# angeris/cfmm-routing-code

Measured on AMD Instinct MI355X. Metric: pool-subproblems/sec to 1e-6 rel-gap; 1e6 pools / 1k tokens; 1/2/4/8 GPU, higher is better.
Workload: dtype f64; 1 GPU; C3: 1000000 pools per GPU (cp2=700000, w2=200000, gn3-8=100000) / 1000 tokens, linear-utility arbitrage, cold-start solve to gap,infeas <= 1e-06; pools_per_gpu=1000000, pools_total=1000000, seed=0, parallelism=single GPU, rccl_ranks=1

## Files before the change

cfmm-routing-code_amd/csrc/cfmm_hip.hip:

```cpp
#include <hip/hip_runtime.h>
#include <dlfcn.h>
#include <algorithm>
#include <cmath>
#include <atomic>
#include <chrono>
#include <condition_variable>
#include <cstdarg>
#include <cstdio>
#include <cstdlib>
#include <cstring>
#include <map>
#include <memory>
#include <set>
#include <mutex>
#include <functional>
#include <limits>
#include <string>
#include <thread>
#include <type_traits>
#include <vector>

#include "../../include/cfmm.h"
#include "kernels.hpp"
#include "iterate.hpp"
// ... 413 lines not shown
            if (!got) {
                std::unique_lock<std::mutex> g(mu_);
                cv_.wait(g, [&]() { return gen_.load(std::memory_order_acquire) != seen; });
            }
            seen = gen_.load(std::memory_order_acquire);
            { std::lock_guard<std::mutex> g(mu_); if (!job_) continue; active_.fetch_add(1, std::memory_order_relaxed); }
            work();
            active_.fetch_sub(1, std::memory_order_release);
        }
    }
    std::mutex mu_, run_mu_;
    std::condition_variable cv_;
    const std::function<void(int)> *job_ = nullptr;
    int njobs_ = 0, nthreads_ = 0;
    std::atomic<int> next_{0}, left_{0}, active_{0};
    std::atomic<unsigned long long> gen_{0};
};

struct UploadScan {
    std::atomic<bool> bad{false};
    std::mutex mu;
    double mxr = 0.0, mnf = 1.0;
    void fold(double mx, double mn) { std::lock_guard<std::mutex> g(mu); mxr = std::max(mxr, mx); mnf = std::min(mnf, mn); }
};
struct Col {
    size_t bytes = 0;
    void **dst = nullptr;
    std::function<void(char *out, size_t off, size_t len)> fill;
    const void *direct = nullptr;
};
template <class F>
void parallel_range(int64_t m, F f)
{
    const int T = m >= (1 << 15) ? HostPool::get().threads() : 1;
    if (T == 1) { f((int64_t)0, m); return; }
    const int64_t part = (m + T - 1) / T;
    HostPool::get().run(T, [&](int t) { const int64_t b = t * part, e = std::min<int64_t>(m, b + part); if (b < e) f(b, e); });
}

template <class T, class P>
inline bool copy_scan(T *out, const T *src, size_t cnt, P pred, T &mx, T &mn)
{
    std::memcpy(out, src, cnt * sizeof(T));
    bool ok0 = true, ok1 = true, ok2 = true, ok3 = true;
    T a0 = mx, a1 = mx, a2 = mx, a3 = mx, b0 = mn, b1 = mn, b2 = mn, b3 = mn;
    size_t i = 0;
    for (; i + 4 <= cnt; i += 4) {
        const T x0 = out[i], x1 = out[i + 1], x2 = out[i + 2], x3 = out[i + 3];
        ok0 &= pred(x0); ok1 &= pred(x1); ok2 &= pred(x2); ok3 &= pred(x3);
        a0 = x0 > a0 ? x0 : a0; a1 = x1 > a1 ? x1 : a1; a2 = x2 > a2 ? x2 : a2; a3 = x3 > a3 ? x3 : a3;
        b0 = x0 < b0 ? x0 : b0; b1 = x1 < b1 ? x1 : b1; b2 = x2 < b2 ? x2 : b2; b3 = x3 < b3 ? x3 : b3;
    }
    for (; i < cnt; ++i) { const T x = out[i]; ok0 &= pred(x); a0 = x > a0 ? x : a0; b0 = x < b0 ? x : b0; }
    mx = std::max(std::max(a0, a1), std::max(a2, a3)); mn = std::min(std::min(b0, b1), std::min(b2, b3));
    return ok0 && ok1 && ok2 && ok3;
}
template <class T, class P>
Col checked_col(const T *src, size_t count, void **dst, UploadScan *scan, int role, P pred)
{
    Col c; c.bytes = count * sizeof(T); c.dst = dst; c.direct = src;
    c.fill = [src, scan, role, pred](char *out, size_t off, size_t len) {
        T mx = T(0), mn = T(1);
        if (role == 2) { mx = std::numeric_limits<T>::lowest(); mn = std::numeric_limits<T>::max(); }
        if (!copy_scan<T>((T *)out, src + off / sizeof(T), len / sizeof(T), pred, mx, mn)) scan->bad.store(true, std::memory_order_relaxed);
        if (role == 0) scan->fold((double)mx, 1.0);
        if (role == 1) scan->fold(0.0, (double)mn);
    };
    return c;
}
Col plain_col(const void *src, size_t bytes, void **dst)
{
    Col c; c.bytes = bytes; c.dst = dst; c.direct = src;
    c.fill = [src](char *out, size_t off, size_t len) { std::memcpy(out, (const char *)src + off, len); };
    return c;
}
template <class T, int K, class P>
inline void transpose_fill(T *o, const T *src, int64_t m, size_t e, size_t cnt, P pred, bool &ok, T &mx)
{
    size_t q = 0;
    int64_t i = (int64_t)(e / K); int j = (int)(e % K);
    for (; q < cnt && j != 0; ++q) { const T x = src[(size_t)j * m + i]; o[q] = x; ok &= pred(x); mx = x > mx ? x : mx; if (++j == K) { j = 0; ++i; } }
    bool okv = true; T mxv = mx;
    for (; q + K <= cnt; q += K, ++i) {
#pragma unroll
        for (int jj = 0; jj < K; ++jj) { const T x = src[(size_t)jj * m + i]; o[q + jj] = x; okv &= pred(x); mxv = x > mxv ? x : mxv; }
    }
    ok &= okv; mx = mxv;
    for (j = 0; q < cnt; ++q, ++j) { const T x = src[(size_t)j * m + i]; o[q] = x; ok &= pred(x); mx = x > mx ? x : mx; }
}
template <class T, class P>
Col transposed_col(const T *src, int k, int64_t m, void **dst, UploadScan *scan, bool track_max, P pred)
{
    Col c; c.bytes = (size_t)k * m * sizeof(T); c.dst = dst;
    c.fill = [src, k, m, scan, track_max, pred](char *out, size_t off, size_t len) {
        T *o = (T *)out;
        const size_t e = off / sizeof(T), cnt = len / sizeof(T);
        bool ok = true; T mx = T(0);
        with_int<2, 8>(k, [&](auto K) { transpose_fill<T, K>(o, src, m, e, cnt, pred, ok, mx); });
        if (!ok) scan->bad.store(true, std::memory_order_relaxed);
        if (track_max) scan->fold((double)mx, 1.0);
    };
    return c;
}
void parallel_fill(const Col &c, char *out, size_t off, size_t len)
{
    const size_t grain = 64u << 10;
    int T = (int)std::min<size_t>((len + grain - 1) / grain, (size_t)HostPool::get().threads());
    if (T <= 1) { c.fill(out, off, len); return; }
    const size_t part = ((len / T) + 63) & ~(size_t)63;
    HostPool::get().run(T, [&](int t) {
        const size_t b = (size_t)t * part, e = (t == T - 1) ? len : std::min(len, b + part);
        if (b < e) c.fill(out + b, off + b, e - b);
    });
}
int upload_arena(cfmm_ctx *ctx, std::vector<Col> &cols, void **arena_out, const UploadScan *scan = nullptr, size_t *total_out = nullptr)
{
    size_t total = 0;
    std::vector<size_t> offs;
    size_t staged = 0;
    for (auto &c : cols) {
        offs.push_back(total); total += (c.bytes + 255) & ~(size_t)255;
        if (c.fill) { if (staged != offs.back()) return fail(ctx, CFMM_E_STATE, "upload: a staged column behind a reserved one"); staged = total; }
    }
    char *base = nullptr;
    static const bool trace = getenv("CFMM_UPLOAD_TRACE") != nullptr;
    auto now = []() { return std::chrono::steady_clock::now(); };
    auto ms = [](std::chrono::steady_clock::time_point a, std::chrono::steady_clock::time_point b) { return std::chrono::duration<double, std::milli>(b - a).count(); };
    const auto tA = now();
    HIP_TRY(ctx, hipMalloc((void **)&base, total + 256));
    if (total_out) *total_out = total;
    const auto tB = now();
    double t_fill = 0.0, t_wait = 0.0, t_enq = 0.0;
    auto bail = [&](hipError_t e, const char *what) { (void)hipStreamSynchronize(ctx->stream); (void)hipFree(base); return fail(ctx, CFMM_E_HIP, "upload: %s -> %s", what, hipGetErrorString(e)); };
    static const bool by_register = getenv("CFMM_UPLOAD") && std::string(getenv("CFMM_UPLOAD")) == "register";
    if (by_register) {
        std::vector<void *> pinned;
        hipError_t e = hipSuccess;
        for (size_t q = 0; q < cols.size() && e == hipSuccess; ++q) {
            if (!cols[q].fill) { *cols[q].dst = base + offs[q]; continue; }
            std::vector<char> tmp(cols[q].bytes);
            cols[q].fill(tmp.data(), 0, cols[q].bytes);
            if (cols[q].direct && cols[q].bytes >= (1u << 20)) {
                e = hipHostRegister(const_cast<void *>(cols[q].direct), cols[q].bytes, hipHostRegisterDefault);
                if (e == hipSuccess) { pinned.push_back(const_cast<void *>(cols[q].direct)); e = hipMemcpyAsync(base + offs[q], cols[q].direct, cols[q].bytes, hipMemcpyHostToDevice, ctx->stream); }
            } else {
                e = hipMemcpy(base + offs[q], tmp.data(), cols[q].bytes, hipMemcpyHostToDevice);
            }
            *cols[q].dst = base + offs[q];
        }
        if (e == hipSuccess) e = hipStreamSynchronize(ctx->stream);
        for (void *h : pinned) (void)hipHostUnregister(h);
        if (e != hipSuccess) return bail(e, "hipHostRegister / copy");
        if (scan && scan->bad.load()) { (void)hipFree(base); return CFMM_E_ARG; }
        *arena_out = base;
        return CFMM_OK;
    }
    std::lock_guard<std::mutex> lock(g_stage.mu);
    if (!g_stage.buf) {
        hipError_t e = hipHostMalloc((void **)&g_stage.buf, STAGE_SLOTS * STAGE_BYTES, hipHostMallocDefault);
        if (e != hipSuccess) { g_stage.buf = nullptr; return bail(e, "hipHostMalloc(staging)"); }
        for (auto &ev : g_stage.ev) { e = hipEventCreateWithFlags(&ev, hipEventDisableTiming); if (e != hipSuccess) return bail(e, "hipEventCreate"); }
    }
    struct Job { size_t q, col_off, len, st_off; };
    int slot = g_stage.next;
    bool *used = g_stage.used;
    std::vector<Job> jobs;
    for (size_t c0 = 0; c0 < staged; c0 += STAGE_BYTES) {
        const size_t clen = std::min(STAGE_BYTES, staged - c0);
        char *st = g_stage.buf + (size_t)slot * STAGE_BYTES;
        jobs.clear();
        for (size_t q = 0; q < cols.size(); ++q) {
            const size_t lo = std::max(offs[q], c0), hi = std::min(offs[q] + cols[q].bytes, c0 + clen);
            if (lo >= hi || !cols[q].fill) continue;
            const size_t grain = 64u << 10;
            for (size_t b = lo; b < hi; b += grain) jobs.push_back({q, b - offs[q], std::min(grain, hi - b), b - c0});
        }
        const auto t0 = now();
        if (used[slot]) { hipError_t e = stage_slot_wait(slot); if (e != hipSuccess) return bail(e, "hipEventSynchronize"); }
        const auto t1 = now();
        HostPool::get().run((int)jobs.size(), [&](int j) { const Job &w = jobs[j]; cols[w.q].fill(st + w.st_off, w.col_off, w.len); });
        const auto t2 = now();
        if (scan && scan->bad.load(std::memory_order_relaxed)) { (void)hipStreamSynchronize(ctx->stream); (void)hipFree(base); return CFMM_E_ARG; }
        hipError_t e = hipMemcpyAsync(base + c0, st, clen, hipMemcpyHostToDevice, ctx->stream);
        if (e == hipSuccess) e = hipEventRecord(g_stage.ev[slot], ctx->stream);
        if (e != hipSuccess) return bail(e, "hipMemcpyAsync");
        t_wait += ms(t0, t1); t_fill += ms(t1, t2); t_enq += ms(t2, now());
        used[slot] = true; g_stage.last[slot] = ctx->stream; slot = (slot + 1) % STAGE_SLOTS;
    }
    for (size_t q = 0; q < cols.size(); ++q) *cols[q].dst = base + offs[q];
    g_stage.next = slot;
    if (trace) fprintf(stderr, "[cfmm upload] %.2f MB: hipMalloc %.3f ms, fill %.3f, wait-for-slot %.3f, enqueue %.3f, total %.3f\n",
                       total / 1e6, ms(tA, tB), t_fill, t_wait, t_enq, ms(tA, now()));
    *arena_out = base;
    return CFMM_OK;
}

int download_staged(cfmm_ctx *ctx, void *host_dst, const void *dev_src, size_t bytes)
{
    if (bytes < (1u << 20)) {
        HIP_TRY(ctx, hipMemcpyAsync(host_dst, dev_src, bytes, hipMemcpyDeviceToHost, ctx->stream));
        HIP_TRY(ctx, hipStreamSynchronize(ctx->stream));
        return CFMM_OK;
    }
    std::lock_guard<std::mutex> lock(g_stage.mu);
    if (!g_stage.buf) {
        HIP_TRY(ctx, hipHostMalloc((void **)&g_stage.buf, STAGE_SLOTS * STAGE_BYTES, hipHostMallocDefault));
        for (auto &ev : g_stage.ev) HIP_TRY(ctx, hipEventCreateWithFlags(&ev, hipEventDisableTiming));
    }
    for (int q = 0; q < STAGE_SLOTS; ++q) if (g_stage.used[q]) { HIP_TRY(ctx, stage_slot_wait(q)); g_stage.used[q] = false; }
    const size_t nchunks = (bytes + STAGE_BYTES - 1) / STAGE_BYTES;
    auto enqueue = [&](size_t c) -> hipError_t {
        const size_t off = c * STAGE_BYTES, len = std::min(STAGE_BYTES, bytes - off);
        const int slot = (int)(c % STAGE_SLOTS);
        hipError_t e = hipMemcpyAsync(g_stage.buf + (size_t)slot * STAGE_BYTES, (const char *)dev_src + off, len, hipMemcpyDeviceToHost, ctx->stream);
        if (e == hipSuccess) e = hipEventRecord(g_stage.ev[slot], ctx->stream);
        return e;
    };
    hipError_t e = hipSuccess;
    for (size_t c = 0; c < std::min<size_t>(nchunks, STAGE_SLOTS - 1) && e == hipSuccess; ++c) e = enqueue(c);
    for (size_t c = 0; c < nchunks && e == hipSuccess; ++c) {
        if (c + STAGE_SLOTS - 1 < nchunks) e = enqueue(c + STAGE_SLOTS - 1);
        if (e != hipSuccess) break;
        const int slot = (int)(c % STAGE_SLOTS);
        e = hipEventSynchronize(g_stage.ev[slot]);
        if (e != hipSuccess) break;
        const size_t off = c * STAGE_BYTES, len = std::min(STAGE_BYTES, bytes - off);
        Col col = plain_col(g_stage.buf + (size_t)slot * STAGE_BYTES, len, nullptr);
        parallel_fill(col, (char *)host_dst + off, 0, len);
    }
    if (e != hipSuccess) { (void)hipStreamSynchronize(ctx->stream); return fail(ctx, CFMM_E_HIP, "read-back -> %s", hipGetErrorString(e)); }
    return CFMM_OK;
}

template <class Launch> int read_back(cfmm_ctx *ctx, const char *who, size_t cnt, double *delta, double *lambda, Launch &&launch)
{
    double *dd = nullptr, *dl = nullptr;
    { int rc = trade_scratch(ctx, cnt, &dd, &dl); if (rc) return rc; }
    launch(dd, dl);
    hipError_t e = hipGetLastError();
    if (e != hipSuccess) return fail(ctx, CFMM_E_HIP, "%s -> %s", who, hipGetErrorString(e));
    if (delta) { int rc = download_staged(ctx, delta, dd, cnt * sizeof(double)); if (rc) return rc; }
    if (lambda) { int rc = download_staged(ctx, lambda, dl, cnt * sizeof(double)); if (rc) return rc; }
    HIP_TRY(ctx, hipStreamSynchronize(ctx->stream));
    return CFMM_OK;
}

void local_extrema(cfmm_ctx *ctx)
{
    ctx->max_reserve = 0.0; ctx->min_fee = 1.0;
    ctx->pools->each([ctx](const auto &r) {
        if (r.b.m) { ctx->max_reserve = std::max(ctx->max_reserve, r.mxr); ctx->min_fee = std::min(ctx->min_fee, r.mnf); }
    });
    ctx->g_max_reserve = ctx->max_reserve;
}

void point_from_caller(cfmm_ctx *ctx)
{
    Point &p = ctx->pt;
    p.have_nu = true; p.hsol_valid = false; p.mu_last = 0.0; p.slo_active = false; p.tr_ovr_valid = false;
}
void point_published(cfmm_ctx *ctx, double mu, bool slo, std::vector<double> *tenders = nullptr)
{
    Point &p = ctx->pt;
    p.have_nu = true; p.hsol_valid = true; p.mu_last = mu; p.slo_active = slo; p.tr_ovr_valid = tenders != nullptr;
    if (tenders) p.tr_ovr.swap(*tenders);
}
void drop_tenders(cfmm_ctx *ctx) { ctx->pt.tr_ovr_valid = false; }
void drop_barrier(cfmm_ctx *ctx) { ctx->pt.mu_last = 0.0; ctx->pt.slo_active = false; }
struct TenderPoint { const double *nu, *slo; double mu; };
TenderPoint tender_point(const cfmm_ctx *ctx)
{
    const route::PointView v = route::point_view(ctx->pt.mu_last, ctx->pt.slo_active);
    return {ctx->nu_acc, v.use_slo ? ctx->sm_slo : nullptr, v.mu};
}
void reserves_moved(cfmm_ctx *ctx)
{
    local_extrema(ctx);
    ctx->g_valid = false; ctx->g_counts_valid = false;
    Point &p = ctx->pt;
    p.hsol_valid = false; p.mu_last = 0.0; p.slo_active = false; p.tr_ovr_valid = false;
}

void pools_changed(cfmm_ctx *ctx)
{
    reserves_moved(ctx);
    ctx->listed_valid = false;
    ctx->pool_gen = ctx->pools->gen.load(std::memory_order_acquire);
}

void pools_seen(cfmm_ctx *ctx)
{
    const unsigned long long g = ctx->pools->gen.load(std::memory_order_acquire);
    if (g == ctx->pool_gen) return;
    ctx->pool_gen = g;
    reserves_moved(ctx);
    for (int k = 0; k < CFMM_POOL_KINDS2; ++k)
        if (ctx->sm_ws[k]) (void)hipMemsetAsync(ctx->sm_ws[k], 0, 2 * (size_t)ctx->sm_ws_m[k] * sizeof(double), ctx->stream);
}

size_t eval_lds_bytes(int n, bool with_d, bool det = false, bool dma = false)
{
    return (size_t)eval_lds_doubles(n, with_d, det) * sizeof(double) + (size_t)(EVAL_THREADS / 64) * 64 * 16 + (dma ? (size_t)(EVAL_THREADS / 64) * STAGE_BYTES : 0);
}
size_t iter_lds_bytes(int n, bool det = false, bool dma = false) { return eval_lds_bytes(n, false, det) + (size_t)iter_extra_lds_doubles(n, dma) * sizeof(double); }
constexpr size_t LDS_MAX = 160 * 1024;
size_t upd_lds_bytes(int ng) { return (size_t)(2 * ng + 16 * 64 + 64 + 32 + 2 * 12 * 16 + 8) * sizeof(double); }

const int kOrder[N_BUCKETS] = {-8, -7, -6, -5, -4, -3, CFMM_POOL_CURVE2, CFMM_POOL_POW2, CFMM_POOL_W2, CFMM_POOL_CP2, CFMM_POOL_SUM2};
static_assert(N_KINDS2 == CFMM_POOL_KINDS2, "kernels.hpp and include/cfmm.h disagree on the two-asset kinds");

void det_scales(cfmm_ctx *ctx, double &sc, double &scd)
{
    const double mr = std::max(ctx->det_ref_reserve > 0.0 ? ctx->det_ref_reserve : (sharded(ctx) ? ctx->g_max_reserve : ctx->max_reserve), 1e-300);
    const double mf = ctx->det_ref_fee > 0.0 ? ctx->det_ref_fee : ctx->min_fee;
    int e = 0;
    (void)std::frexp(mr / std::max(mf, 1e-3), &e);
    sc = std::ldexp(1.0, 84 - e);
    (void)std::frexp(mr * std::max(ctx->nu_max, 1e-300), &e);
    scd = std::ldexp(1.0, 84 - e);
}

static bool wide_tiles(const cfmm_ctx *ctx)
{
    static const int wide_mode = getenv("CFMM_WIDE") ? atoi(getenv("CFMM_WIDE")) : -1;
    return !CFMM_STAGED_WALK && !ctx->det && (wide_mode > 0 || (wide_mode < 0 && ctx->pools->r2[CFMM_POOL_CP2].b.m >= 8000000));
}
EvalArgs make_eval_args(cfmm_ctx *ctx, bool stable, int only = 0x7fffffff, bool big = true)
{
    EvalArgs a = {};
    for (int k = 0; k < CFMM_POOL_KINDS2; ++k) a.b2[k] = ctx->pools->r2[k].b;
    a.b2[CFMM_POOL_SUM2].flags = ctx->flags2;
    for (int k = 3; k <= CFMM_MAX_POOL_SIZE; ++k) a.bn[k - 3] = ctx->pools->rn[k].b;
    a.wide = (big && wide_tiles(ctx)) ? 1 : 0;
    long long tiles = 0;
    for (int q = 0; q < N_BUCKETS; ++q) {
        const int code = kOrder[q];
        const long long m = code < 0 ? ctx->pools->rn[-code].b.m : ctx->pools->r2[code].b.m;
        const int wt = (code == CFMM_POOL_CP2 && a.wide) ? WT_WIDE : wave_tile_pools(code);
        if ((only == 0x7fffffff || only == code) && ((code >= 0 && heavy_kind(code)) == stable)) tiles += (m + wt - 1) / wt;
        a.tile_end[q] = (int)tiles;
    }
    a.ntiles = (int)tiles;
    a.n = ctx->n; a.nslices = ctx->nslices;
    a.nu = ctx->nu; a.acc = ctx->acc; a.ts = ctx->ts;
    a.acc_l = ctx->acc_l;
    det_scales(ctx, a.det_scale, a.det_scale_d);
    return a;
}

void eval_geometry(cfmm_ctx *ctx, int ntiles, int &grid, int &threads)
{
    const int slots = ctx->cus * ctx->eval_blocks_per_cu * ctx->eval_grid_mult;
    int wpb = (ntiles + slots - 1) / slots;
    wpb = wpb < 1 ? 1 : (wpb > EVAL_THREADS / 64 ? EVAL_THREADS / 64 : wpb);
    threads = 64 * wpb;
    grid = (ntiles + wpb - 1) / wpb;
    if (grid > slots) grid = slots;
    if (grid < 1) grid = 1;
}

static bool pingpong_on(const cfmm_ctx *ctx)
{
    static const int mode = getenv("CFMM_PINGPONG") ? atoi(getenv("CFMM_PINGPONG")) : -1;
    if (mode >= 0) return mode != 0;
    double b2 = 0.0, bn = 0.0;
    for (int k = 0; k < CFMM_POOL_KINDS2; ++k) b2 += (double)ctx->pools->r2[k].b.m * ((k == CFMM_POOL_CP2 || k == CFMM_POOL_SUM2) ? 32.0 : 40.0);
    for (int k = 3; k <= CFMM_MAX_POOL_SIZE; ++k) bn += (double)ctx->pools->rn[k].b.m * (20.0 + 20.0 * k);
    return bn <= 0.1 * (b2 + bn);
}

static bool stream_nt(const cfmm_ctx *ctx)
{
    static const int mode = getenv("CFMM_NT") ? atoi(getenv("CFMM_NT")) : -1;
    if (mode >= 0) return mode != 0 && !ctx->det;
    double bytes = 0.0;
    for (int k = 0; k < CFMM_POOL_KINDS2; ++k) if (!heavy_kind(k)) bytes += (double)ctx->pools->r2[k].b.m * ((k == CFMM_POOL_CP2 || k == CFMM_POOL_SUM2) ? 32.0 : 40.0);
    for (int k = 3; k <= CFMM_MAX_POOL_SIZE; ++k) bytes += (double)ctx->pools->rn[k].b.m * (20.0 + 20.0 * k);
    return !ctx->det && bytes > 2.0 * 256.0 * 1048576.0;
}
static int large_set_mode(const cfmm_ctx *ctx)
{
    if (ctx->det) return 0;
    if (stream_nt(ctx)) return 1;
    bool mirror = false;
    for (auto &r : ctx->pools->r2) mirror = mirror || r.cmem != nullptr;
    return (mirror || wide_tiles(ctx)) ? 2 : 0;
}
static bool eval_dma(const cfmm_ctx *ctx, bool with_d) { return CFMM_STAGED_WALK && ctx->tile_dma && !ctx->det && eval_lds_bytes(ctx->n, with_d, false, true) <= LDS_MAX; }
static bool iter_dma(const cfmm_ctx *ctx) { return CFMM_STAGED_WALK && ctx->tile_dma && !ctx->det && iter_lds_bytes(ctx->n, false, true) <= LDS_MAX; }

template <bool WITH_D, bool STABLE>
void launch_eval(cfmm_ctx *ctx, const EvalArgs &a_in, hipStream_t stream = nullptr)
{
    if (a_in.ntiles == 0) return;
    if (!stream) stream = ctx->stream;
    EvalArgs a = a_in;
    if (pingpong_on(ctx)) { a.rev = ctx->walk_parity[STABLE ? 1 : 0] & 1; ctx->walk_parity[STABLE ? 1 : 0] ^= 1; }
    int grid, threads;
    eval_geometry(ctx, a.ntiles, grid, threads);
    if (ctx->det) hipLaunchKernelGGL((eval_kernel<WITH_D, STABLE, true>), dim3(grid), dim3(threads), eval_lds_bytes(ctx->n, WITH_D, true), stream, a);
#if CFMM_STAGED_WALK
    else if (!STABLE && eval_dma(ctx, WITH_D)) hipLaunchKernelGGL((eval_kernel<WITH_D, false, false, true>), dim3(grid), dim3(threads), eval_lds_bytes(ctx->n, WITH_D, false, true), stream, a);
#endif
    else if (!STABLE && large_set_mode(ctx) == 1) hipLaunchKernelGGL((eval_kernel<WITH_D, false, false, false, 1>), dim3(grid), dim3(threads), eval_lds_bytes(ctx->n, WITH_D), stream, a);
    else if (!STABLE && large_set_mode(ctx) == 2) hipLaunchKernelGGL((eval_kernel<WITH_D, false, false, false, 2>), dim3(grid), dim3(threads), eval_lds_bytes(ctx->n, WITH_D), stream, a);
    else hipLaunchKernelGGL((eval_kernel<WITH_D, STABLE>), dim3(grid), dim3(threads), eval_lds_bytes(ctx->n, WITH_D), stream, a);
}

int det_finish(cfmm_ctx *ctx, double *out, const double *nu, bool with_d)
{
    const int n = ctx->n;
    if (sharded(ctx)) { int rc = all_reduce(ctx, ctx->acc_l, (size_t)(with_d ? 6 : 3) * n, NCCL_INT64, NCCL_SUM); if (rc) return rc; }
    double sc, scd;
    det_scales(ctx, sc, scd);
    hipLaunchKernelGGL(det_fold_kernel, dim3(1), dim3(1024), 0, ctx->stream, ctx->acc_l, nu, out, n, 1.0 / sc, 1.0 / scd, with_d ? 1 : 0);
    return CFMM_OK;
}

int64_t heavy_pools(const cfmm_ctx *ctx)
{
    int64_t m = 0;
    for (int k = 0; k < CFMM_POOL_KINDS2; ++k) if (heavy_kind(k)) m += ctx->pools->r2[k].b.m;
    return m;
}

int64_t table_pools(const cfmm_ctx *ctx)
{
    int64_t m = 0;
    for (auto &row : ctx->pools->rg) for (auto &r : row) m += r.b.m;
    return m;
}
int64_t table_sum_pools(const cfmm_ctx *ctx)
{
    int64_t m = 0;
    for (auto &r : ctx->pools->rg[CFMM_POOLK_SUM]) m += r.b.m;
    return m;
}
int64_t extra_launch_pools(const cfmm_ctx *ctx) { return heavy_pools(ctx) + table_pools(ctx); }

TableArgs make_table_args(cfmm_ctx *ctx, const double *nu, double *acc)
{
    TableArgs a = {};
    long long tiles = 0;
    for (int q = 0; q < 2; ++q)
        for (int k = 2; k <= CFMM_MAX_POOL_SIZE; ++k) {
            const BucketG &b = ctx->pools->rg[q == 0 ? CFMM_POOLK_STABLE : CFMM_POOLK_SUM][k].b;
            (q == 0 ? a.bs : a.bq)[k - 2] = b;
            if (q == 1) a.qflags[k - 2] = ctx->flagsG[k];
            const int P = 64 / k;
            tiles += (b.m + P - 1) / P;
            a.tile_end[7 * q + k - 2] = (int)tiles;
        }
    a.ntiles = (int)tiles; a.n = ctx->n; a.nslices = ctx->nslices;
    static const bool warm_off = getenv("CFMM_TABLE_WARM") && atoi(getenv("CFMM_TABLE_WARM")) == 0;
    a.warm = (ctx->det || warm_off) ? 0 : 1;
    a.nu = nu; a.acc = acc; a.acc_l = ctx->acc_l;
    det_scales(ctx, a.det_scale, a.det_scale_d);
    static const double ftol = getenv("CFMM_TABLE_FTOL") ? atof(getenv("CFMM_TABLE_FTOL")) : 1e-9;
    a.ftol = ftol;
    return a;
}
template <bool WITH_D>
void launch_table_evals(cfmm_ctx *ctx, const double *nu, double *acc, hipStream_t stream = nullptr, double *const *ws_row = nullptr)
{
    TableArgs a = make_table_args(ctx, nu, acc);
    if (a.ntiles == 0) return;
    if (!stream) stream = ctx->stream;
    if (ws_row) for (int q = 0; q < 7; ++q) { a.bs[q].ws = ws_row[q]; if (!ws_row[q] && a.bs[q].m) a.warm = 0; }
    const int waves = std::min(GT_THREADS / 64, a.ntiles);
    int grid = (a.ntiles + waves - 1) / waves;
    static const int gmult = getenv("CFMM_TABLE_GRID_MULT") ? std::max(1, atoi(getenv("CFMM_TABLE_GRID_MULT"))) : 1;
    grid = std::min(grid, gmult * ctx->cus);
    const size_t lds = table_lds_bytes(ctx->n, WITH_D, ctx->det, waves);
    if (ctx->det) hipLaunchKernelGGL((table_eval_kernel<WITH_D, true>), dim3(grid), dim3(64 * waves), lds, stream, a);
    else hipLaunchKernelGGL((table_eval_kernel<WITH_D, false>), dim3(grid), dim3(64 * waves), lds, stream, a);
}

template <bool WITH_D>
void launch_all_evals(cfmm_ctx *ctx)
{
    launch_eval<WITH_D, false>(ctx, make_eval_args(ctx, false));
    if (heavy_pools(ctx) > 0) launch_eval<WITH_D, true>(ctx, make_eval_args(ctx, true));
    if (table_pools(ctx) > 0) launch_table_evals<WITH_D>(ctx, ctx->nu, ctx->acc);
}

template <class F>
int set_lds_attr(cfmm_ctx *ctx, F f, size_t bytes)
{
    if (bytes > 160 * 1024) return CFMM_OK;
    HIP_TRY(ctx, hipFuncSetAttribute((const void *)f, hipFuncAttributeMaxDynamicSharedMemorySize, (int)bytes));
    return CFMM_OK;
}

int set_all_lds_attrs_uncached(cfmm_ctx *ctx);
int set_all_lds_attrs(cfmm_ctx *ctx)
{
    static std::mutex mu;
    static int done_n[64] = {};
    std::lock_guard<std::mutex> g(mu);
    const int d = ctx->device & 63;
    if (ctx->n <= done_n[d]) return CFMM_OK;
    int rc = set_all_lds_attrs_uncached(ctx);
    if (rc == CFMM_OK) done_n[d] = ctx->n;
    return rc;
}
int set_all_lds_attrs_uncached(cfmm_ctx *ctx)
{
    const size_t e0 = eval_lds_bytes(ctx->n, false), e1 = eval_lds_bytes(ctx->n, true);
    int rc;
    if ((rc = set_lds_attr(ctx, eval_kernel<false, false>, e0))) return rc;
    if ((rc = set_lds_attr(ctx, eval_kernel<true, false>, e1))) return rc;
    if ((rc = set_lds_attr(ctx, eval_kernel<false, true>, e0))) return rc;
    if ((rc = set_lds_attr(ctx, eval_kernel<true, true>, e1))) return rc;
    if ((rc = set_lds_attr(ctx, eval_kernel<false, false, false, false, 1>, e0))) return rc;
    if ((rc = set_lds_attr(ctx, eval_kernel<true, false, false, false, 1>, e1))) return rc;
    if ((rc = set_lds_attr(ctx, eval_kernel<false, false, false, false, 2>, e0))) return rc;
    if ((rc = set_lds_attr(ctx, eval_kernel<true, false, false, false, 2>, e1))) return rc;
#if CFMM_STAGED_WALK
    if (eval_lds_bytes(ctx->n, false, false, true) <= LDS_MAX && (rc = set_lds_attr(ctx, eval_kernel<false, false, false, true>, eval_lds_bytes(ctx->n, false, false, true)))) return rc;
    if (eval_lds_bytes(ctx->n, true, false, true) <= LDS_MAX && (rc = set_lds_attr(ctx, eval_kernel<true, false, false, true>, eval_lds_bytes(ctx->n, true, false, true)))) return rc;
#endif
    if ((rc = set_lds_attr(ctx, update_kernel<false>, upd_lds_bytes(ctx->n)))) return rc;
    if ((rc = set_lds_attr(ctx, update_reg_kernel<512, 8, 2>, upd_lds_bytes(ctx->n)))) return rc;
    if ((rc = set_lds_attr(ctx, update_reg_kernel<512, 4, 4>, upd_lds_bytes(ctx->n)))) return rc;
    if ((rc = set_lds_attr(ctx, update_reg_kernel<256, 8, 4>, upd_lds_bytes(ctx->n)))) return rc;
    if ((rc = set_lds_attr(ctx, update_gram_kernel<512, 2>, upd_lds_bytes(ctx->n)))) return rc;
    if ((rc = set_lds_attr(ctx, start_kernel<false>, upd_lds_bytes(ctx->n)))) return rc;
    if ((rc = set_lds_attr(ctx, update_kernel<true>, upd_lds_bytes(ctx->n)))) return rc;
    if ((rc = set_lds_attr(ctx, update_reg_kernel<512, 8, 2, true>, upd_lds_bytes(ctx->n)))) return rc;
    if ((rc = set_lds_attr(ctx, update_reg_kernel<512, 8, 2, false, true>, upd_lds_bytes(ctx->n)))) return rc;
    if ((rc = set_lds_attr(ctx, update_reg_kernel<512, 4, 4, true>, upd_lds_bytes(ctx->n)))) return rc;
    if ((rc = set_lds_attr(ctx, update_gram_kernel<512, 2, true>, upd_lds_bytes(ctx->n)))) return rc;
    if ((rc = set_lds_attr(ctx, start_kernel<true>, upd_lds_bytes(ctx->n)))) return rc;
    if ((rc = set_lds_attr(ctx, eval_batch_kernel, batch_lds_bytes(ctx->n, batch_capacity(ctx->n))))) return rc;
    if ((rc = set_lds_attr(ctx, eval_batch_heavy_kernel, batch_lds_bytes(ctx->n, batch_capacity(ctx->n))))) return rc;
    if ((rc = set_lds_attr(ctx, table_batch_eval_kernel, table_batch_lds_bytes(ctx->n, batch_capacity(ctx->n), GT_THREADS / 64)))) return rc;
    if ((rc = set_lds_attr(ctx, table_eval_kernel<false, false>, table_lds_bytes(ctx->n, false, false, GT_THREADS / 64)))) return rc;
    if ((rc = set_lds_attr(ctx, table_eval_kernel<true, false>, table_lds_bytes(ctx->n, true, false, GT_THREADS / 64)))) return rc;
    if ((rc = set_lds_attr(ctx, table_newton_kernel<false>, table_newton_lds_bytes(ctx->n, GT_THREADS / 64)))) return rc;
    if ((rc = set_lds_attr(ctx, table_newton_kernel<true>, table_newton_lds_bytes(ctx->n, GT_THREADS / 64)))) return rc;
    if (ctx->n <= TINY_N && (rc = set_lds_attr(ctx, solve_tiny_kernel<false>, (size_t)tiny_lds_doubles(ctx->n) * sizeof(double)))) return rc;
    if (ctx->n <= TINY_N && (rc = set_lds_attr(ctx, solve_tiny_kernel<true>, (size_t)tiny_lds_doubles(ctx->n) * sizeof(double)))) return rc;
    const size_t il = iter_lds_bytes(ctx->n);
    if ((rc = set_lds_attr(ctx, iter_kernel<ITER_E_SMALL, false, false>, il))) return rc;
    if ((rc = set_lds_attr(ctx, iter_kernel<ITER_E_SMALL, false, true>, il))) return rc;
    if ((rc = set_lds_attr(ctx, iter_kernel<2, false, false>, il))) return rc;
    if ((rc = set_lds_attr(ctx, iter_kernel<2, false, true>, il))) return rc;
    if ((rc = set_lds_attr(ctx, iter_kernel<2, false, false, false, 1>, il))) return rc;
    if ((rc = set_lds_attr(ctx, iter_kernel<2, false, true, false, 1>, il))) return rc;
    if ((rc = set_lds_attr(ctx, iter_kernel<2, false, false, false, 2>, il))) return rc;
    if ((rc = set_lds_attr(ctx, iter_kernel<2, false, true, false, 2>, il))) return rc;
#if CFMM_STAGED_WALK
    if (ctx->n <= 2 * EVAL_THREADS && iter_lds_bytes(ctx->n, false, true) <= LDS_MAX) {
        const size_t ilm = iter_lds_bytes(ctx->n, false, true);
        if ((rc = set_lds_attr(ctx, iter_kernel<2, false, false, true>, ilm))) return rc;
        if ((rc = set_lds_attr(ctx, iter_kernel<2, false, true, true>, ilm))) return rc;
    }
#endif
    if (eval_lds_bytes(ctx->n, true, true) <= 160 * 1024) {
        if ((rc = set_lds_attr(ctx, eval_kernel<false, false, true>, eval_lds_bytes(ctx->n, false, true)))) return rc;
        if ((rc = set_lds_attr(ctx, eval_kernel<true, false, true>, eval_lds_bytes(ctx->n, true, true)))) return rc;
        if ((rc = set_lds_attr(ctx, eval_kernel<false, true, true>, eval_lds_bytes(ctx->n, false, true)))) return rc;
        if ((rc = set_lds_attr(ctx, eval_kernel<true, true, true>, eval_lds_bytes(ctx->n, true, true)))) return rc;
        if ((rc = set_lds_attr(ctx, table_eval_kernel<false, true>, table_lds_bytes(ctx->n, false, true, GT_THREADS / 64)))) return rc;
        if ((rc = set_lds_attr(ctx, table_eval_kernel<true, true>, table_lds_bytes(ctx->n, true, true, GT_THREADS / 64)))) return rc;
        const size_t ild = iter_lds_bytes(ctx->n, true);
        if ((rc = set_lds_attr(ctx, iter_kernel<ITER_E_SMALL, true, false>, ild))) return rc;
        if ((rc = set_lds_attr(ctx, iter_kernel<ITER_E_SMALL, true, true>, ild))) return rc;
        if ((rc = set_lds_attr(ctx, iter_kernel<2, true, false>, ild))) return rc;
        if ((rc = set_lds_attr(ctx, iter_kernel<2, true, true>, ild))) return rc;
    }
    return CFMM_OK;
}

UpdArgs make_upd_args(cfmm_ctx *ctx, const cfmm_opts &o)
{
    UpdArgs a;
    a.n = ctx->n; a.ng = ctx->ng; a.M = o.memory; a.nslices = (sharded(ctx) || ctx->det) ? 1 : ctx->nslices;
    a.acc = ctx->acc;
    a.c = ctx->c; a.h = ctx->h; a.off = ctx->off; a.glo = ctx->glo; a.ghi = ctx->ghi;
    a.ctype = ctx->ctype; a.grp = ctx->grp;
    a.gptr = ctx->ng != ctx->n ? ctx->gptr : nullptr; a.gmem = ctx->gmem; a.tie_tmp = ctx->tie_tmp;
    a.nu = ctx->nu; a.nu_acc = ctx->nu_acc; a.psi_acc = ctx->psi_acc; a.psi_t = ctx->psi_t;
    a.s = ctx->s; a.s_t = ctx->s_t; a.Gs = ctx->Gs; a.Gs_t = ctx->Gs_t; a.d = ctx->d; a.Ds = ctx->Ds;
    a.S = ctx->S; a.Y = ctx->Y; a.rho = ctx->rho;
    a.st = ctx->st;
    a.tol_gap = o.tol_gap; a.tol_infeas = o.tol_infeas; a.armijo = o.armijo; a.max_step = o.max_step;
    a.max_evals = o.max_evals; a.pg_rule = o.pg_rule; a.ts = ctx->ts;
    a.batch = nullptr; a.hstat = nullptr; a.pool_flags = nullptr;
    return a;
}

bool tiny_applies(cfmm_ctx *ctx, const EvalArgs &ea, const cfmm_opts &o)
{
    return ctx->tiny_path && !ctx->general_utility && !sharded(ctx) && !ctx->det && extra_launch_pools(ctx) == 0 && ea.ntiles >= 1 &&
           ea.ntiles <= TINY_MAX_TILES && ctx->n <= TINY_N && o.memory <= MAX_MEMORY;
}

bool fused_applies(cfmm_ctx *ctx, const cfmm_opts &o)
{
    return ctx->fused && !ctx->general_utility && ctx->ng == ctx->n && ctx->n <= 2 * EVAL_THREADS && o.memory <= ITER_MM;
}

size_t acc_set_doubles(cfmm_ctx *ctx) { return (size_t)ctx->nslices * acc_stride(ctx->n); }

IterArgs make_iter_args(cfmm_ctx *ctx, const cfmm_opts &o)
{
    IterArgs a = {};
    a.ev = make_eval_args(ctx, false);
    a.ev.nu = nullptr; a.ev.acc = nullptr;
    a.n = ctx->n; a.M = o.memory; a.nread = ((sharded(ctx) && !rccl_unfolded(ctx)) || ctx->det) ? 1 : ctx->nslices; a.phase = 0;
    a.xvs = iter_xvs(ctx->n); a.max_evals = o.max_evals; a.pg_rule = o.pg_rule;
    a.plain = ctx->plain ? 1 : 0;
    a.acc3 = ctx->acc3; a.acc_set = (long long)acc_set_doubles(ctx);
    a.xs = ctx->xs3; a.xs_set = (long long)XS_VECS * a.xvs;
    a.st3 = ctx->st3;
    a.c = ctx->c; a.h = ctx->h; a.glo = ctx->glo; a.ghi = ctx->ghi; a.ctype = ctx->ctype;
    a.Ds = ctx->Ds;
    a.nu = ctx->nu; a.nu_acc = ctx->nu_acc; a.psi_acc = ctx->psi_acc;
    a.tol_gap = o.tol_gap; a.tol_infeas = o.tol_infeas; a.armijo = o.armijo; a.max_step = o.max_step;
    a.hstat = ctx->hstat_d;
    return a;
}

bool oneshot_runahead(cfmm_ctx *ctx)
{
    return ctx->os_ready && !ctx->det && (size_t)acc_stride(ctx->n) <= ctx->os_cap && extra_launch_pools(ctx) == 0;
}

int enqueue_fused_iteration(cfmm_ctx *ctx, const IterArgs &base, int t)
{
    IterArgs a = base;
    a.phase = t % 3; a.launch = t;
    a.ev.rev = pingpong_on(ctx) ? (t & 1) : 0;
    const int n = ctx->n, E = (n <= EVAL_THREADS && ITER_E_SMALL == 1) ? 1 : 2;
    int grid, threads;
    {
        const int slots = ctx->cus * ctx->iter_blocks_per_cu * ctx->eval_grid_mult;
        int wpb = (a.ev.ntiles + slots - 1) / slots;
        wpb = wpb < 1 ? 1 : (wpb > EVAL_THREADS / 64 ? EVAL_THREADS / 64 : wpb);
        const int need = (n + 64 * E - 1) / (64 * E);
        if (wpb < need) wpb = need;
        threads = 64 * wpb;
        grid = (a.ev.ntiles + wpb - 1) / wpb;
        if (grid > slots) grid = slots;
        if (grid < 1) grid = 1;
    }
    const bool dma = iter_dma(ctx);
    const int big = dma ? 0 : large_set_mode(ctx);
    const size_t lds = iter_lds_bytes(n, ctx->det, dma);
    const dim3 g(grid), b(threads);
#if CFMM_STAGED_WALK
#define ITER_LAUNCH_DMA if (dma) { if (a.plain) hipLaunchKernelGGL((iter_kernel<2, false, true, true>), g, b, lds, ctx->stream, a); else hipLaunchKernelGGL((iter_kernel<2, false, false, true>), g, b, lds, ctx->stream, a); }
#else
#define ITER_LAUNCH_DMA if (false) { }
#endif
#define ITER_LAUNCH(EE) do { \
        ITER_LAUNCH_DMA else if (big == 1) { if (a.plain) hipLaunchKernelGGL((iter_kernel<2, false, true, false, 1>), g, b, lds, ctx->stream, a); else hipLaunchKernelGGL((iter_kernel<2, false, false, false, 1>), g, b, lds, ctx->stream, a); } \
        else if (big == 2) { if (a.plain) hipLaunchKernelGGL((iter_kernel<2, false, true, false, 2>), g, b, lds, ctx->stream, a); else hipLaunchKernelGGL((iter_kernel<2, false, false, false, 2>), g, b, lds, ctx->stream, a); } \
        else if (ctx->det) { if (a.plain) hipLaunchKernelGGL((iter_kernel<EE, true, true>), g, b, lds, ctx->stream, a); else hipLaunchKernelGGL((iter_kernel<EE, true, false>), g, b, lds, ctx->stream, a); } \
        else { if (a.plain) hipLaunchKernelGGL((iter_kernel<EE, false, true>), g, b, lds, ctx->stream, a); else hipLaunchKernelGGL((iter_kernel<EE, false, false>), g, b, lds, ctx->stream, a); } } while (0)
    if (E == 1) ITER_LAUNCH(ITER_E_SMALL); else ITER_LAUNCH(2);
#undef ITER_LAUNCH
    double *acc_p = ctx->acc3 + (size_t)a.phase * acc_set_doubles(ctx);
    if (heavy_pools(ctx) > 0) {
        EvalArgs es = make_eval_args(ctx, true);
        es.nu = ctx->nu; es.acc = acc_p;
        launch_eval<false, true>(ctx, es);
    }
    if (table_pools(ctx) > 0) launch_table_evals<false>(ctx, ctx->nu, acc_p);
    if (ctx->det) return det_finish(ctx, acc_p, ctx->nu, false);
    if (sharded(ctx)) {
        const DevState *stop = oneshot_runahead(ctx) ? ctx->st3 + a.phase : nullptr;
        const int len = acc_arb(n) + 1;
        if (rccl_unfolded(ctx)) return all_reduce(ctx, acc_p, (size_t)(ctx->nslices - 1) * acc_stride(n) + len, NCCL_FLOAT64, NCCL_SUM);
        return all_reduce(ctx, acc_p, (size_t)len, NCCL_FLOAT64, NCCL_SUM, stop, ctx->nslices);
    }
    return CFMM_OK;
}

void launch_update(cfmm_ctx *ctx, const UpdArgs &ua)
{
    const int n = ctx->n;
    const size_t lds = upd_lds_bytes(ctx->ng);
    auto thr = [n](int E) { return 64 * ((n + 64 * E - 1) / (64 * E)); };
    const int ug = ctx->upd_grid;
    static const bool gen_generic = getenv("CFMM_UTILITY_GENERIC") && atoi(getenv("CFMM_UTILITY_GENERIC")) != 0;
    if (ctx->general_utility && !ctx->upd_generic && !gen_generic && n <= 1024 && ctx->ng == ctx->n) {
        hipLaunchKernelGGL((update_reg_kernel<512, 8, 2, false, true>), dim3(1), dim3(thr(2)), lds, ctx->stream, ua);
        return;
    }
    const int v = (ctx->upd_generic || ctx->general_utility) ? 9 : ctx->upd_variant;
    if (v == 0 && n <= 1024 && ua.M <= GRAM_MM)
        hipLaunchKernelGGL((update_gram_kernel<512, 2>), dim3(ug), dim3(thr(2)), lds, ctx->stream, ua);
    else if ((v == 0 || v == 3) && n <= 1024)
        hipLaunchKernelGGL((update_reg_kernel<512, 8, 2>), dim3(ug), dim3(thr(2)), lds, ctx->stream, ua);
    else if ((v == 0 || v == 1 || v == 3) && n <= 2048 && ua.M <= 4)
        hipLaunchKernelGGL((update_reg_kernel<512, 4, 4>), dim3(ug), dim3(thr(4)), lds, ctx->stream, ua);
    else if (v == 2 && n <= 1024)
        hipLaunchKernelGGL((update_reg_kernel<256, 8, 4>), dim3(1), dim3(thr(4)), lds, ctx->stream, ua);
    else
        hipLaunchKernelGGL(update_kernel<false>, dim3(1), dim3(UPD_THREADS), lds, ctx->stream, ua);
}

template <bool WITH_D>
int enqueue_iteration(cfmm_ctx *ctx, const UpdArgs &ua)
{
    launch_all_evals<WITH_D>(ctx);
    if (ctx->det) { int rc = det_finish(ctx, ctx->acc, ctx->nu, WITH_D); if (rc) return rc; }
    else if (sharded(ctx)) {
        const int len = WITH_D ? acc_stride(ctx->n) : acc_arb(ctx->n) + 1;
        hipLaunchKernelGGL(fold_kernel, dim3((len + 255) / 256), dim3(256), 0, ctx->stream, ctx->acc, ctx->n,
                           ctx->nslices, WITH_D ? 1 : 0, (const DevState *)nullptr);
        int rc = all_reduce(ctx, ctx->acc, (size_t)len, NCCL_FLOAT64, NCCL_SUM); if (rc) return rc;
    }
    launch_update(ctx, ua);
    return CFMM_OK;
}

int bounds_into_mirror(cfmm_ctx *ctx)
{
    const int n = ctx->n, ng = ctx->ng;
    double *lo = (double *)(ctx->util_h + ((char *)ctx->glo - (char *)ctx->c)), *hi = (double *)(ctx->util_h + ((char *)ctx->ghi - (char *)ctx->c));
    const int j = sweep::group_bounds(n, ctx->hc.data(), ctx->hctype.data(), ctx->hgrp.data(), ctx->hoff.data(), ng, lo, hi);
    if (j >= 0) return fail(ctx, CFMM_E_ARG, "token %d: CFMM_FREE needs c > 0", j);
    return CFMM_OK;
}

int recompute_bounds(cfmm_ctx *ctx)
{
    const int ng = ctx->ng;
    { int rc = bounds_into_mirror(ctx); if (rc) return rc; }
    const size_t olo = (size_t)((char *)ctx->glo - (char *)ctx->c), ohi = (size_t)((char *)ctx->ghi - (char *)ctx->c);
    HIP_TRY(ctx, hipMemcpyAsync(ctx->glo, ctx->util_h + olo, ng * sizeof(double), hipMemcpyHostToDevice, ctx->stream));
    HIP_TRY(ctx, hipMemcpyAsync(ctx->ghi, ctx->util_h + ohi, ng * sizeof(double), hipMemcpyHostToDevice, ctx->stream));
    HIP_TRY(ctx, hipStreamSynchronize(ctx->stream));
    return CFMM_OK;
}

void drop_graph(cfmm_ctx *ctx)
{
    if (ctx->gexec) { (void)hipGraphExecDestroy(ctx->gexec); ctx->gexec = nullptr; }
    ctx->g_valid = false;
}

int build_graph(cfmm_ctx *ctx, const cfmm_opts &o)
{
    drop_graph(ctx);
    const UpdArgs ua = make_upd_args(ctx, o);
    hipGraph_t graph = nullptr;
    stage_ring_drain(ctx->stream);
    HIP_TRY(ctx, hipStreamBeginCapture(ctx->stream, hipStreamCaptureModeThreadLocal));
    int rc = CFMM_OK;
    if (fused_applies(ctx, o)) {
        const IterArgs ia = make_iter_args(ctx, o);
        for (int it = 0; it < o.iters_per_graph && rc == CFMM_OK; ++it) rc = enqueue_fused_iteration(ctx, ia, it + 1);
    } else
    for (int it = 0; it < o.iters_per_graph && rc == CFMM_OK; ++it) rc = enqueue_iteration<false>(ctx, ua);
    hipError_t e = hipStreamEndCapture(ctx->stream, &graph);
    if (rc != CFMM_OK) { if (graph) (void)hipGraphDestroy(graph); return rc; }
    if (e != hipSuccess) return fail(ctx, CFMM_E_HIP, "hipStreamEndCapture -> %s", hipGetErrorString(e));
    e = hipGraphInstantiate(&ctx->gexec, graph, nullptr, nullptr, 0);
    (void)hipGraphDestroy(graph);
    if (e != hipSuccess) return fail(ctx, CFMM_E_HIP, "hipGraphInstantiate -> %s", hipGetErrorString(e));
    ctx->g_opts = o; ctx->g_valid = true;
    return CFMM_OK;
}

bool same_opts(const cfmm_opts &a, const cfmm_opts &b) { return std::memcmp(&a, &b, sizeof(cfmm_opts)) == 0; }

}

extern "C" int cfmm_eval_dual(cfmm_ctx *ctx, const double *nu, double *arb_sum, double *psi, double *diag);
extern "C" int64_t cfmm_pool_count(cfmm_ctx *ctx);
extern "C" int64_t cfmm_eval_bytes(cfmm_ctx *ctx);

namespace {

int hess_nr(int n) { return (n + 2 * CH_NB - 1) / (2 * CH_NB) * (2 * CH_NB); }
int hess_ld(int n) { return hess_nr(n) + CH_NB; }

int launch_factor(cfmm_ctx *ctx, int n, bool info_zeroed = false)
{
    const int nr = hess_nr(n), ld = hess_ld(n), nrows = nr + 1, nbk = nr / CH_NB;
    if (!info_zeroed) HIP_TRY(ctx, hipMemsetAsync(ctx->sm_info, 0, 4 * sizeof(int), ctx->stream));
    const bool inv = ctx->inverse_factor && ctx->Winv;
    if (ctx->chol_pairs) {
        const size_t lds = (size_t)CH2_LDS_DOUBLES * sizeof(double);
        int arrived = 0;
        for (int c0 = 0; c0 < nr; c0 += 2 * CH_NB) {
            const int below = nrows - c0 - 2 * CH_NB;
            const int npanel = 1 + (below + CH2_ROWS - 1) / CH2_ROWS;
            int ntiles = 0;
            if (c0 > 0 && nr - c0 - 2 * CH_NB > 0) { const int T = (below + 63) / 64; ntiles = T * (T + 1) / 2; }
            const int qb = c0 / CH_NB - 1;
            const int ntw = (inv && c0 > 0) ? (nbk - 1 - qb) * (qb + 1) : 0;
            const int nside = std::min(ntw + ntiles, std::max(ctx->cus - npanel, 1));
            arrived += npanel - 1;
            hipLaunchKernelGGL(chol_step2_kernel, dim3(npanel + nside), dim3(256), lds, ctx->stream, ctx->H, ld, nrows, nr, c0, npanel, ctx->Dinv, ctx->sm_info,
                               npanel + ntw, ctx->Winv, ctx->Rinv, nr, 0, ntw + ntiles, arrived);
        }
        if (inv && nbk >= 2)
            hipLaunchKernelGGL(chol_step2_kernel, dim3(nbk - 1), dim3(256), lds, ctx->stream, ctx->H, ld, nrows, nr, nr, 0, ctx->Dinv, ctx->sm_info,
                               nbk - 1, ctx->Winv, ctx->Rinv, nr, 1, nbk - 1, 0);
        HIP_TRY(ctx, hipGetLastError());
        return CFMM_OK;
    }
    int arrived = 0;
    for (int k1 = 0; k1 < nr; k1 += CH_NB) {
        const int below = nrows - k1 - CH_NB;
        const int npanel = 1 + (below + 63) / 64;
        arrived += npanel - 1;
        int ntiles = 0;
        if (k1 > 0 && nr - k1 - CH_NB > 0) { const int T = (below + 63) / 64; ntiles = T * (T + 1) / 2; }
        const int q = k1 / CH_NB - 1;
        const int ntw = (inv && q >= 0) ? (nbk - 1 - q) * (q + 1) : 0;
        hipLaunchKernelGGL(chol_step_kernel, dim3(npanel + ntw + ntiles), dim3(256), 0, ctx->stream, ctx->H, ld, nrows, nr, k1, npanel, ctx->Dinv, ctx->sm_info,
                           npanel + ntw, ctx->Winv, ctx->Rinv, nr, arrived);
    }
    HIP_TRY(ctx, hipGetLastError());
    return CFMM_OK;
}
int launch_backsolve(cfmm_ctx *ctx, int n, double *x)
{
    const int nr = hess_nr(n), ld = hess_ld(n);
    if (ctx->inverse_factor && ctx->Winv) {
        hipLaunchKernelGGL(chol_wt_kernel, dim3((nr + CH_WT_THREADS / 64 - 1) / (CH_WT_THREADS / 64)), dim3(CH_WT_THREADS), (size_t)nr * sizeof(double), ctx->stream,
                           (const double *)(ctx->H + nr), ld, nr, n, (const double *)ctx->Dinv, (const double *)ctx->Winv, (const double *)ctx->Rinv, nr, x);
        HIP_TRY(ctx, hipGetLastError());
        return CFMM_OK;
    }
    hipLaunchKernelGGL(chol_back_kernel, dim3(1), dim3(CH_SOLVE_THREADS), (size_t)(nr + CH_NB + 2 * CH_NB * CH_NB) * sizeof(double), ctx->stream,
                       (const double *)ctx->H, ld, nr, n, (const double *)ctx->Dinv, x);
    HIP_TRY(ctx, hipGetLastError());
    return CFMM_OK;
}
int launch_chord(cfmm_ctx *ctx, int n, const double *g, double *x)
{
    const int nr = hess_nr(n);
    if (!(ctx->inverse_factor && ctx->Winv)) return fail(ctx, CFMM_E_STATE, "chord step: no inverse factor (CFMM_BACKSUB=classic)");
    hipLaunchKernelGGL(chol_w_kernel, dim3((nr + CH_W_ROWS - 1) / CH_W_ROWS), dim3(CH_W_THREADS), 0, ctx->stream,
                       g, nr, n, (const double *)ctx->Dinv, (const double *)ctx->Winv, (const double *)ctx->Rinv, nr, ctx->chord_y);
    hipLaunchKernelGGL(chol_wt_kernel, dim3((nr + CH_WT_THREADS / 64 - 1) / (CH_WT_THREADS / 64)), dim3(CH_WT_THREADS), (size_t)nr * sizeof(double), ctx->stream,
                       (const double *)ctx->chord_y, 1, nr, n, (const double *)ctx->Dinv, (const double *)ctx->Winv, (const double *)ctx->Rinv, nr, x);
    HIP_TRY(ctx, hipGetLastError());
    return CFMM_OK;
}
int launch_cholesky(cfmm_ctx *ctx, int n, double *x, bool info_zeroed = false)
{
    int rc = launch_factor(ctx, n, info_zeroed);
    return rc ? rc : launch_backsolve(ctx, n, x);
}

bool newton_supported(cfmm_ctx *ctx, const char **why)
{
    if (ctx->ng != ctx->n) { *why = "price ties are set"; return false; }
    if (smooth_lds_bytes(ctx->n, true) > LDS_MAX) { *why = "too many tokens for the second-order path's LDS tiles (psi, Hessian diagonal and pair cache: 5792 tokens)"; return false; }
    *why = "";
    return true;
}

bool near_linear_pools(cfmm_ctx *ctx) { return ctx->g_stable >= CFMM_AUTO_NEWTON_MIN_STABLE; }

int refresh_global_counts(cfmm_ctx *ctx)
{
    if (sharded(ctx) && ctx->g_counts_valid) return CFMM_OK;
    ctx->g_total = cfmm_pool_count(ctx);
    ctx->g_stable = ctx->pools->r2[CFMM_POOL_CURVE2].b.m;
    ctx->g_table = table_sum_pools(ctx);
    local_extrema(ctx);
    if (!sharded(ctx)) return CFMM_OK;
    {
        double mx[2] = {ctx->max_reserve, 1.0 / ctx->min_fee};
        double *dm = ctx->psi_t + 2;
        HIP_TRY(ctx, hipMemcpyAsync(dm, mx, sizeof mx, hipMemcpyHostToDevice, ctx->stream));
        { int rc = all_reduce(ctx, dm, 2, NCCL_FLOAT64, NCCL_MAX); if (rc) return rc; }
        HIP_TRY(ctx, hipMemcpyAsync(mx, dm, sizeof mx, hipMemcpyDeviceToHost, ctx->stream));
        HIP_TRY(ctx, hipStreamSynchronize(ctx->stream));
        ctx->g_max_reserve = mx[0]; ctx->min_fee = 1.0 / mx[1];
    }
    double cnt[3] = {(double)ctx->g_total, (double)ctx->g_stable, (double)ctx->g_table};
    double *dv = ctx->psi_t;
    HIP_TRY(ctx, hipMemcpyAsync(dv, cnt, sizeof cnt, hipMemcpyHostToDevice, ctx->stream));
    { int rc = all_reduce(ctx, dv, 3, NCCL_FLOAT64, NCCL_SUM); if (rc) return rc; }
    HIP_TRY(ctx, hipMemcpyAsync(cnt, dv, sizeof cnt, hipMemcpyDeviceToHost, ctx->stream));
    HIP_TRY(ctx, hipStreamSynchronize(ctx->stream));
    ctx->g_total = (int64_t)cnt[0]; ctx->g_stable = (int64_t)cnt[1]; ctx->g_table = (int64_t)cnt[2];
    ctx->g_counts_valid = true;
    return CFMM_OK;
}

constexpr size_t PIN_FLAG_BACK = 8;
double *pin_scratch(cfmm_ctx *ctx, size_t doubles)
{
    doubles = std::max(doubles, 8 * (size_t)ctx->n + 64);
    if (doubles > ctx->pin_cap) {
        if (ctx->pin) { (void)hipHostFree(ctx->pin); ctx->pin = nullptr; ctx->pin_dev = nullptr; ctx->pin_cap = 0; }
        if (hipHostMalloc((void **)&ctx->pin, doubles * sizeof(double), hipHostMallocCoherent) != hipSuccess) { ctx->pin = nullptr; return nullptr; }
        if (hipHostGetDevicePointer((void **)&ctx->pin_dev, ctx->pin, 0) != hipSuccess) { (void)hipHostFree(ctx->pin); ctx->pin = nullptr; ctx->pin_dev = nullptr; return nullptr; }
        ctx->pin_cap = doubles;
        std::memset(ctx->pin, 0, doubles * sizeof(double));
    }
    return ctx->pin;
}
inline unsigned long long *io_flag_host(cfmm_ctx *ctx) { return reinterpret_cast<unsigned long long *>(ctx->pin + 8 * (size_t)ctx->n + 64 - PIN_FLAG_BACK); }
template <class T> inline T *pin_device(cfmm_ctx *ctx, T *host) { return reinterpret_cast<T *>(reinterpret_cast<char *>(ctx->pin_dev) + (reinterpret_cast<char *>(host) - reinterpret_cast<char *>(ctx->pin))); }

struct IoList {
    IoArgs a{};
    size_t maxb = 0;
    void copy(void *dst, const void *src, size_t bytes) { a.j[a.njobs++] = IoJob{dst, src, (unsigned long long)((bytes + 7) & ~(size_t)7)}; maxb = std::max(maxb, bytes); }
    void zero(void *dst, size_t bytes) { copy(dst, nullptr, bytes); }
};
int launch_io(cfmm_ctx *ctx, IoList &l, bool publish)
{
    if (l.a.njobs < 1 || l.a.njobs > IO_MAX_JOBS) return fail(ctx, CFMM_E_STATE, "hand-off: %d jobs", l.a.njobs);
    unsigned grid = 1;
    if (publish) { l.a.flag = pin_device(ctx, io_flag_host(ctx)); l.a.seq = ++ctx->io_seq; }
    else grid = (unsigned)std::min<size_t>(std::max<size_t>((l.maxb + 256 * 64 - 1) / (256 * 64), 1), 2 * (size_t)ctx->cus);
    hipLaunchKernelGGL(io_kernel, dim3(grid), dim3(256), 0, ctx->stream, l.a);
    HIP_TRY(ctx, hipGetLastError());
    return CFMM_OK;
}
int wait_io(cfmm_ctx *ctx)
{
    volatile unsigned long long *f = io_flag_host(ctx);
    const unsigned long long want = ctx->io_seq;
    const auto t0 = std::chrono::steady_clock::now();
    for (unsigned spin = 1;; ++spin) {
        if (*f == want) { std::atomic_thread_fence(std::memory_order_acquire); return CFMM_OK; }
        __builtin_ia32_pause();
        if ((spin & 0x3fff) == 0 && std::chrono::duration<double>(std::chrono::steady_clock::now() - t0).count() > 2.0) break;
    }
    HIP_TRY(ctx, hipStreamSynchronize(ctx->stream));
    if (*f == want) { std::atomic_thread_fence(std::memory_order_acquire); return CFMM_OK; }
    return fail(ctx, CFMM_E_HIP, "hand-off: the stream drained without the kernel's flag (%llu, expected %llu)", (unsigned long long)*f, want);
}

struct HandOff {
    enum Kind { Down, Up, Zero, ZeroLeanOnly };
    struct Job { Kind kind; void *dst; const void *src; size_t bytes; };
    cfmm_ctx *ctx;
    Job j[IO_MAX_JOBS];
    int nj = 0;
    explicit HandOff(cfmm_ctx *c) : ctx(c) {}
    void down(void *dev, const void *pinned, size_t bytes) { j[nj++] = Job{Down, dev, pinned, bytes}; }
    void up(void *pinned, const void *dev, size_t bytes) { j[nj++] = Job{Up, pinned, dev, bytes}; }
    void zero(void *dev, size_t bytes) { j[nj++] = Job{Zero, dev, nullptr, bytes}; }
    void zero_lean_only(void *dev, size_t bytes) { j[nj++] = Job{ZeroLeanOnly, dev, nullptr, bytes}; }
    int run(bool publish)
    {
        if (ctx->lean_io) {
            IoList l;
            for (int i = 0; i < nj; ++i)
                l.copy(j[i].kind == Up ? pin_device(ctx, j[i].dst) : j[i].dst, j[i].kind == Down ? pin_device(ctx, const_cast<void *>(j[i].src)) : j[i].src, j[i].bytes);
            const int rc = launch_io(ctx, l, publish);
            return rc || !publish ? rc : wait_io(ctx);
        }
        for (int i = 0; i < nj; ++i) {
            if (j[i].kind == Down) HIP_TRY(ctx, hipMemcpyAsync(j[i].dst, j[i].src, j[i].bytes, hipMemcpyHostToDevice, ctx->stream));
            if (j[i].kind == Up) HIP_TRY(ctx, hipMemcpyAsync(j[i].dst, j[i].src, j[i].bytes, hipMemcpyDeviceToHost, ctx->stream));
            if (j[i].kind == Zero) HIP_TRY(ctx, hipMemsetAsync(j[i].dst, 0, j[i].bytes, ctx->stream));
        }
        if (publish) HIP_TRY(ctx, hipStreamSynchronize(ctx->stream));
        return CFMM_OK;
// ... 2959 lines not shown
    const route::AuditStage &st = R.st = route::audit_stage(R.counts, R.kink, own);
    if (st.half == route::slot2(CFMM_POOL_SUM2)) return fail(ctx, CFMM_E_ARG, "audit_trades: own names one array of the constant-sum bucket without the other");
    if (st.half >= 0) return fail(ctx, CFMM_E_ARG, "audit_trades: own names one array of the %d-asset constant-sum bucket without the other", route::slot_name(st.half).k);
    { int rc = tender_room(ctx, st.len); if (rc) return rc; }
    auto send = [&](size_t off, const double *src, size_t cnt) { return cnt ? hipMemcpyAsync(ctx->tender_dev + off, src, cnt * sizeof(double), hipMemcpyHostToDevice, ctx->stream) : hipSuccess; };
    if (R.kink) HIP_TRY(ctx, send(0, ctx->pt.tr_ovr.data(), R.tl.two_asset()));
    const size_t m2 = (size_t)R.counts.m[route::slot2(CFMM_POOL_SUM2)];
    if (st.own2) { HIP_TRY(ctx, send(st.off_own2, own->sum2_delta, 2 * m2)); HIP_TRY(ctx, send(st.off_own2 + 2 * m2, own->sum2_lambda, 2 * m2)); }
    for (int k = 2; k <= CFMM_MAX_POOL_SIZE; ++k)
        if (st.ownk[k]) {
            const size_t cnt = (size_t)k * R.counts.m[route::slotG(CFMM_POOLK_SUM, k)];
            HIP_TRY(ctx, send(st.off_ownk[k], own->sumk_delta[k], cnt)); HIP_TRY(ctx, send(st.off_ownk[k] + cnt, own->sumk_lambda[k], cnt));
        }
    return CFMM_OK;
}

int audit_launches(AuditRun &R)
{
    cfmm_ctx *ctx = R.ctx;
    const route::AuditStage &st = R.st;
    AuditArgs a;
    a.n = ctx->n; a.sc = R.sc; a.tol = R.tol;
    a.limbs = (unsigned long long *)(ctx->audit_dev + R.sp.limbs);
    AuditRec *recs = (AuditRec *)(ctx->audit_dev + R.sp.recs), *parts = (AuditRec *)(ctx->audit_dev + R.sp.parts);
    const size_t lds = 3 * (size_t)ctx->n * sizeof(unsigned long long);
    const TenderPoint p = tender_point(ctx);
    const double *dev = ctx->tender_dev;
    const dim3 blk(AU_THREADS);
    ctx->audit_reordered = 0;
    each_bucket(R.ps, [&](auto &r, int q, auto FAMILY, auto KIND, auto K) {
        auto b = r.b;
        const dim3 grid(audit_grid(ctx, b.m));
        a.rec = recs + q; a.part = parts + (size_t)q * AU_GRID_MAX;
        if constexpr (FAMILY == 0) {
            if (KIND == CFMM_POOL_SUM2) b.flags = ctx->flags2;
            const double *ov = (KIND == CFMM_POOL_SUM2 && st.own2) ? dev + st.off_own2 : (R.kink ? dev + R.tl.off2[KIND] : nullptr);
            ctx->audit_reordered += b.perm != nullptr;
            hipLaunchKernelGGL(audit2_kernel<KIND>, grid, blk, lds, ctx->stream, b, p.nu, p.slo, p.mu, ov, a);
        } else if constexpr (FAMILY == 1) {
            ctx->audit_reordered += b.perm != nullptr;
            hipLaunchKernelGGL(auditN_kernel<K>, grid, blk, lds, ctx->stream, b, p.nu, p.slo, a);
        } else {
            const int *fl = KIND == CFMM_POOLK_SUM ? ctx->flagsG[K] : nullptr;
            const double *ov = (KIND == CFMM_POOLK_SUM && st.ownk[K]) ? dev + st.off_ownk[K] : nullptr;
            hipLaunchKernelGGL((auditG_kernel<KIND, K>), grid, blk, lds, ctx->stream, b, fl, p.nu, p.slo, p.mu, ov, a);
        }
    });
    HIP_TRY(ctx, hipGetLastError());
    return CFMM_OK;
}
int audit_pass(AuditRun &R)
{
    cfmm_ctx *ctx = R.ctx;
    double scd;
    det_scales(ctx, R.sc, scd);
    HIP_TRY(ctx, hipMemsetAsync(ctx->audit_dev, 0, R.sp.parts, ctx->stream));
    return timed_pass(ctx, ctx->audit_timed, &ctx->audit_sec, [&] { return audit_launches(R); }, [&] {
        HIP_TRY(ctx, hipMemcpyAsync(ctx->audit_host, ctx->audit_dev, R.sp.parts, hipMemcpyDeviceToHost, ctx->stream));
        return (int)CFMM_OK;
    });
}

void audit_report(AuditRun &R, cfmm_audit *out, double *psi, uint64_t *limbs)
{
    cfmm_ctx *ctx = R.ctx;
    const int n = ctx->n;
    const AuditRec *res = (const AuditRec *)(ctx->audit_host + R.sp.recs);
    const unsigned long long *hl = (const unsigned long long *)(ctx->audit_host + R.sp.limbs);
    const route::AuditFold f = route::fold_audit(res, R.counts);
    const route::SlotName worst = route::slot_name(f.worst);
    out->fixed_exponent = route::fixed_exponent(R.sc);
    out->pools = f.pools; out->pools_trading = f.trading; out->pools_violating = f.violating; out->legs_out_of_range = f.oor;
    out->worst_family = worst.family; out->worst_kind = worst.kind; out->worst_k = worst.k; out->worst_pos = f.worst_pos;
    out->min_slack = f.min_slack; out->min_tender = f.min_tender; out->min_leg = f.min_leg;
    if (limbs) std::memcpy(limbs, hl, 3 * (size_t)n * sizeof(uint64_t));
    std::vector<double> hp((size_t)n);
    route::psi_from_limbs(hl, n, out->fixed_exponent, hp.data());
    if (psi) std::memcpy(psi, hp.data(), (size_t)n * sizeof(double));
    if (!ctx->have_utility) return;
    const route::PsiWorth w = route::psi_worth(hp.data(), n, ctx->hc.data(), ctx->hh.data(), ctx->hctype.data(), ctx->max_reserve);
    out->value = w.value; out->infeas = w.infeas;
}
}

int cfmm_audit_trades(cfmm_ctx *ctx, const cfmm_audit_tenders *own, double tol_pool, cfmm_audit *out, double *psi, uint64_t *limbs)
{
    const char *who = "audit_trades";
    if (!ctx) return CFMM_E_ARG;
    if (!out) return fail(ctx, CFMM_E_ARG, "%s: out is NULL", who);
    audit_blank(out);
    if (sharded(ctx)) return fail(ctx, CFMM_E_UNSUPPORTED, "%s: pool-sharded contexts are not served (audit the shards' tenders on the host)", who);
    if (ctx->n > AU_MAX_TOKENS) return fail(ctx, CFMM_E_LIMIT, "%s: %d tokens exceed the workgroup's tile of 3 n 64-bit limbs (n <= %d)", who, ctx->n, AU_MAX_TOKENS);
    PoolEntry entry(ctx); HIP_TRY(ctx, entry.device);
    if (!ctx->pt.have_nu) return fail(ctx, CFMM_E_STATE, "%s: no prices yet (cfmm_set_nu or a solve first)", who);
    const route::Counts counts = bucket_counts(entry.ps);
    AuditRun R{ctx, entry.ps, tol_pool > 0.0 ? tol_pool : 1e-9, counts, route::trade_layout(counts), route::audit_span(ctx->n, AU_GRID_MAX), ctx->pt.tr_ovr_valid, {}, 0.0};
    { int rc = audit_reserve(R); if (rc) return rc; }
    { int rc = audit_stage_tenders(R, own); if (rc) return rc; }
    { int rc = audit_pass(R); if (rc) return rc; }
    audit_report(R, out, psi, limbs);
    return CFMM_OK;
}

int cfmm_debug_audit_launch(cfmm_ctx *ctx, int timed, int grid, double *out2)
{
    if (!ctx) return CFMM_E_ARG;
    if (grid < 0 || grid > AU_GRID_MAX) return fail(ctx, CFMM_E_ARG, "debug_audit_launch: grid %d is outside 0 (unchanged), 1 .. %d", grid, AU_GRID_MAX);
    ctx->audit_timed = timed != 0;
    if (grid > 0) ctx->audit_grid = grid;
    if (out2) { out2[0] = ctx->audit_sec; out2[1] = (double)ctx->audit_reordered; }
    return CFMM_OK;
}

int cfmm_comm_unique_id(void *uid128)
{
    if (!uid128) return CFMM_E_ARG;
    std::string err;
    if (!g_rccl.load(err)) return fail(nullptr, CFMM_E_RCCL, "%s", err.c_str());
    ncclUniqueId id;
    int rc = g_rccl.GetUniqueId(&id);
    if (rc != 0) return fail(nullptr, CFMM_E_RCCL, "ncclGetUniqueId failed (%d)", rc);
    std::memcpy(uid128, &id, sizeof id);
    return CFMM_OK;
}

int cfmm_comm_init(cfmm_ctx *ctx, int n_ranks, int rank, const void *uid128)
{
    if (!ctx || n_ranks < 1 || rank < 0 || rank >= n_ranks || !uid128) return ctx ? fail(ctx, CFMM_E_ARG, "comm_init: bad arguments") : CFMM_E_ARG;
    HIP_TRY(ctx, hipSetDevice(ctx->device));
    { int rc_ = settle(ctx); if (rc_) return rc_; }
    std::string err;
    if (!g_rccl.load(err)) return fail(ctx, CFMM_E_RCCL, "%s", err.c_str());
    ncclUniqueId id;
    std::memcpy(&id, uid128, sizeof id);
    int rc = g_rccl.CommInitRank(&ctx->comm, n_ranks, id, rank);
    if (rc != 0) return fail(ctx, CFMM_E_RCCL, "ncclCommInitRank -> %s", g_rccl.GetErrorString ? g_rccl.GetErrorString(rc) : "error");
    ctx->n_ranks = n_ranks; ctx->rank = rank;
    ctx->g_valid = false; ctx->g_counts_valid = false;
    rc = g_rccl.AllReduce(ctx->acc, ctx->acc, (size_t)acc_stride(ctx->n), NCCL_FLOAT64, NCCL_SUM, ctx->comm, ctx->stream);
    if (rc != 0) return fail(ctx, CFMM_E_RCCL, "warm-up ncclAllReduce -> %s", g_rccl.GetErrorString ? g_rccl.GetErrorString(rc) : "error");
    HIP_TRY(ctx, hipStreamSynchronize(ctx->stream));
    return CFMM_OK;
}

int cfmm_set_deterministic(cfmm_ctx *ctx, int on)
{
    if (!ctx) return CFMM_E_ARG;
    if (on && eval_lds_bytes(ctx->n, true, true) > 160 * 1024)
        return fail(ctx, CFMM_E_LIMIT, "set_deterministic: %d tokens exceed the LDS tile of the reproducible mode (7 n doubles)", ctx->n);
    if ((on != 0) != ctx->det) { ctx->g_valid = false; ctx->g_counts_valid = false; }
    ctx->det = on != 0;
    return CFMM_OK;
}

int cfmm_debug_eval_limbs(cfmm_ctx *ctx, const double *nu, double ref_reserve, double ref_fee, uint64_t *limbs)
{
    if (!ctx || !nu || !limbs) return CFMM_E_ARG;
    PoolEntry entry(ctx); HIP_TRY(ctx, entry.device);
    const int n = ctx->n;
    if (eval_lds_bytes(n, true, true) > 160 * 1024) return fail(ctx, CFMM_E_LIMIT, "debug_eval_limbs: too many tokens for the reproducible mode");
    for (int j = 0; j < n; ++j) if (!(nu[j] > 0.0) || !std::isfinite(nu[j])) return fail(ctx, CFMM_E_ARG, "debug_eval_limbs: nu[%d] is not a positive finite price", j);
    { int rc = refresh_global_counts(ctx); if (rc) return rc; }
    const bool was = ctx->det;
    ctx->det = true; ctx->det_ref_reserve = ref_reserve; ctx->det_ref_fee = ref_fee;
    hipError_t e = hipMemcpyAsync(ctx->nu, nu, n * sizeof(double), hipMemcpyHostToDevice, ctx->stream);
    if (e == hipSuccess) e = hipMemsetAsync(ctx->nu + n, 0, sizeof(double), ctx->stream);
    if (e == hipSuccess) e = hipMemsetAsync(ctx->acc_l, 0, 6 * (size_t)n * sizeof(unsigned long long), ctx->stream);
    if (e == hipSuccess) { launch_all_evals<false>(ctx); e = hipGetLastError(); }
    if (e == hipSuccess) e = hipMemcpyAsync(limbs, ctx->acc_l, 3 * (size_t)n * sizeof(uint64_t), hipMemcpyDeviceToHost, ctx->stream);
    if (e == hipSuccess) e = hipMemsetAsync(ctx->acc_l, 0, 6 * (size_t)n * sizeof(unsigned long long), ctx->stream);
    if (e == hipSuccess) e = hipStreamSynchronize(ctx->stream);
    ctx->det = was; ctx->det_ref_reserve = 0.0; ctx->det_ref_fee = 0.0;
    if (e != hipSuccess) return fail(ctx, CFMM_E_HIP, "debug_eval_limbs -> %s", hipGetErrorString(e));
    return CFMM_OK;
}

int cfmm_debug_scatter_limbs(cfmm_ctx *ctx, int64_t count, const int32_t *tok, const double *y, double ref_reserve, double ref_fee, uint64_t *limbs)
{
    if (!ctx || !tok || !y || !limbs || count < 1 || count > (1 << 24)) return ctx ? fail(ctx, CFMM_E_ARG, "debug_scatter_limbs: 1 <= count <= 2^24") : CFMM_E_ARG;
    if (!(ref_reserve > 0.0) || !(ref_fee > 0.0)) return fail(ctx, CFMM_E_ARG, "debug_scatter_limbs: the reference reserve and fee must be positive");
    const int n = ctx->n;
    const double save_r = ctx->det_ref_reserve, save_f = ctx->det_ref_fee;
    ctx->det_ref_reserve = ref_reserve; ctx->det_ref_fee = ref_fee;
    double sc, scd;
    det_scales(ctx, sc, scd);
    ctx->det_ref_reserve = save_r; ctx->det_ref_fee = save_f;
    for (int64_t i = 0; i < count; ++i) {
        if (tok[i] < 0 || tok[i] >= n) return fail(ctx, CFMM_E_ARG, "debug_scatter_limbs: tok[%lld] = %d is not a token", (long long)i, tok[i]);
        if (!(std::fabs(y[i] * sc) < 0x1p95)) return fail(ctx, CFMM_E_ARG, "debug_scatter_limbs: y[%lld] is outside the split's range", (long long)i);
    }
    HIP_TRY(ctx, hipSetDevice(ctx->device));
    { int rc = settle(ctx); if (rc) return rc; }
    const size_t lb = 3 * (size_t)n * sizeof(unsigned long long), yb = (size_t)count * sizeof(double), tb = (size_t)count * sizeof(int32_t);
    char *buf = nullptr;
    HIP_TRY(ctx, hipMalloc((void **)&buf, lb + yb + tb));
    unsigned long long *dL = (unsigned long long *)buf;
    double *dy = (double *)(buf + lb);
    int *dt = (int *)(buf + lb + yb);
    hipError_t e = hipMemsetAsync(dL, 0, lb, ctx->stream);
    if (e == hipSuccess) e = hipMemcpyAsync(dy, y, yb, hipMemcpyHostToDevice, ctx->stream);
    if (e == hipSuccess) e = hipMemcpyAsync(dt, tok, tb, hipMemcpyHostToDevice, ctx->stream);
    if (e == hipSuccess) {
        hipLaunchKernelGGL(debug_scatter_kernel, dim3((unsigned)((count + 255) / 256)), dim3(256), 0, ctx->stream, dL, n, sc, (const int *)dt, (const double *)dy,
                           (long long)count);
        e = hipGetLastError();
    }
    if (e == hipSuccess) e = hipMemcpyAsync(limbs, dL, lb, hipMemcpyDeviceToHost, ctx->stream);
    const hipError_t es = hipStreamSynchronize(ctx->stream);
    if (e == hipSuccess) e = es;
    (void)hipFree(buf);
    if (e != hipSuccess) return fail(ctx, CFMM_E_HIP, "debug_scatter_limbs -> %s", hipGetErrorString(e));
    return CFMM_OK;
}

static int oneshot_alloc(cfmm_ctx *ctx)
{
    if (ctx->os_mail) return CFMM_OK;
    ctx->os_cap = (size_t)std::max(acc_stride(ctx->n), 6 * ctx->n) + 8;
    HIP_TRY(ctx, hipMalloc((void **)&ctx->os_mail, oneshot_alloc_bytes(ctx->os_cap)));
    HIP_TRY(ctx, hipMemsetAsync(ctx->os_mail, 0, oneshot_alloc_bytes(ctx->os_cap), ctx->stream));
    HIP_TRY(ctx, hipStreamSynchronize(ctx->stream));
    return CFMM_OK;
}

void *cfmm_oneshot_mailbox(cfmm_ctx *ctx)
{
    if (!ctx || hipSetDevice(ctx->device) != hipSuccess || oneshot_alloc(ctx) != CFMM_OK) return nullptr;
    return ctx->os_mail;
}

int cfmm_oneshot_export(cfmm_ctx *ctx, void *handle64)
{
    if (!ctx || !handle64) return CFMM_E_ARG;
    HIP_TRY(ctx, hipSetDevice(ctx->device));
    { int rc_ = settle(ctx); if (rc_) return rc_; }
    { int rc = oneshot_alloc(ctx); if (rc) return rc; }
    hipIpcMemHandle_t h;
    static_assert(sizeof(hipIpcMemHandle_t) == 64, "IPC handle size");
    HIP_TRY(ctx, hipIpcGetMemHandle(&h, ctx->os_mail));
    std::memcpy(handle64, &h, sizeof h);
    return CFMM_OK;
}

int cfmm_oneshot_attach(cfmm_ctx *ctx, int n_ranks, int rank, void *const *mailboxes)
{
    if (!ctx || !mailboxes || n_ranks < 1 || n_ranks > ONESHOT_MAX_RANKS || rank < 0 || rank >= n_ranks)
        return ctx ? fail(ctx, CFMM_E_ARG, "oneshot_attach: %d ranks (at most %d), rank %d", n_ranks, ONESHOT_MAX_RANKS, rank) : CFMM_E_ARG;
    HIP_TRY(ctx, hipSetDevice(ctx->device));
    { int rc_ = settle(ctx); if (rc_) return rc_; }
    { int rc = oneshot_alloc(ctx); if (rc) return rc; }
    if (ctx->comm && ctx->n_ranks != n_ranks) return fail(ctx, CFMM_E_STATE, "oneshot_attach: the RCCL communicator has %d ranks", ctx->n_ranks);
    for (int r = 0; r < n_ranks; ++r) {
        ctx->os_peers[r] = r == rank ? ctx->os_mail : (unsigned long long *)mailboxes[r];
        if (!ctx->os_peers[r]) return fail(ctx, CFMM_E_ARG, "oneshot_attach: mailbox of rank %d is NULL", r);
    }
    ctx->n_ranks = n_ranks; ctx->rank = rank;
    HIP_TRY(ctx, hipMemsetAsync(ctx->os_mail, 0, oneshot_alloc_bytes(ctx->os_cap), ctx->stream));
    HIP_TRY(ctx, hipStreamSynchronize(ctx->stream));
    ctx->os_ready = true; ctx->g_valid = false; ctx->g_counts_valid = false;
    return CFMM_OK;
}

int cfmm_oneshot_import(cfmm_ctx *ctx, int n_ranks, int rank, const void *handles)
{
    if (!ctx || !handles || n_ranks < 1 || n_ranks > ONESHOT_MAX_RANKS || rank < 0 || rank >= n_ranks) return ctx ? fail(ctx, CFMM_E_ARG, "oneshot_import: bad arguments") : CFMM_E_ARG;
    HIP_TRY(ctx, hipSetDevice(ctx->device));
    void *ptrs[ONESHOT_MAX_RANKS] = {};
    for (int r = 0; r < n_ranks; ++r) {
        if (r == rank) continue;
        hipIpcMemHandle_t h;
        std::memcpy(&h, (const char *)handles + 64 * (size_t)r, sizeof h);
        void *p = nullptr;
        hipError_t e = hipIpcOpenMemHandle(&p, h, hipIpcMemLazyEnablePeerAccess);
        if (e != hipSuccess) return fail(ctx, CFMM_E_HIP, "oneshot_import: hipIpcOpenMemHandle(rank %d) -> %s", r, hipGetErrorString(e));
        ctx->os_opened.push_back(p);
        ptrs[r] = p;
    }
    return cfmm_oneshot_attach(ctx, n_ranks, rank, ptrs);
}

int cfmm_oneshot_enable(cfmm_ctx *ctx, int on)
{
    if (!ctx) return CFMM_E_ARG;
    if (on && !ctx->os_peers[ctx->rank]) return fail(ctx, CFMM_E_STATE, "oneshot_enable: no mailboxes attached (cfmm_oneshot_import / _attach first)");
    if (!on && !ctx->comm && ctx->os_ready) return fail(ctx, CFMM_E_STATE, "oneshot_enable(0): no RCCL communicator to fall back on");
    HIP_TRY(ctx, hipSetDevice(ctx->device));
    { int rc_ = settle(ctx); if (rc_) return rc_; }
    HIP_TRY(ctx, hipStreamSynchronize(ctx->stream));
    if ((on != 0) != ctx->os_ready) drop_graph(ctx);
    ctx->os_ready = on != 0; ctx->g_counts_valid = false;
    return CFMM_OK;
}

int cfmm_selftest(cfmm_ctx *ctx)
{
    if (!ctx) return CFMM_E_ARG;
    HIP_TRY(ctx, hipSetDevice(ctx->device));
    { int rc_ = settle(ctx); if (rc_) return rc_; }
    int *d = nullptr, h = -1;
    HIP_TRY(ctx, hipMalloc((void **)&d, sizeof(int)));
    HIP_TRY(ctx, hipMemsetAsync(d, 0, sizeof(int), ctx->stream));
    hipLaunchKernelGGL(selftest_kernel, dim3(1), dim3(64), 0, ctx->stream, d);
    hipLaunchKernelGGL(selftest_gram_kernel, dim3(1), dim3(64), 0, ctx->stream, d);
    hipLaunchKernelGGL(selftest_log_kernel, dim3(1), dim3(64), 0, ctx->stream, d);
    hipLaunchKernelGGL(selftest_generic_kernel, dim3(1), dim3(64), 0, ctx->stream, d);
    hipLaunchKernelGGL(selftest_table_kernel, dim3(1), dim3(64), 0, ctx->stream, d);
    hipError_t e = hipMemcpyAsync(&h, d, sizeof(int), hipMemcpyDeviceToHost, ctx->stream);
    if (e == hipSuccess) e = hipStreamSynchronize(ctx->stream);
    (void)hipFree(d);
    if (e != hipSuccess) return fail(ctx, CFMM_E_HIP, "selftest -> %s", hipGetErrorString(e));
    if (h != 0) return fail(ctx, CFMM_E_NUMERIC, "selftest: %d results of the cross-lane reductions / the fast logarithm / the generic pool solver are wrong on this device / ROCm", h);
    return CFMM_OK;
}

int cfmm_debug_timers(cfmm_ctx *ctx, int64_t *out64)
{
    if (!ctx || !out64) return CFMM_E_ARG;
    HIP_TRY(ctx, hipSetDevice(ctx->device));
    { int rc_ = settle(ctx); if (rc_) return rc_; }
    HIP_TRY(ctx, hipStreamSynchronize(ctx->stream));
    HIP_TRY(ctx, hipMemcpy(out64, ctx->ts, (64 + 8 * 4096 + 2048) * sizeof(int64_t), hipMemcpyDeviceToHost));
    HIP_TRY(ctx, hipMemset(ctx->ts, 0, (64 + 8 * 4096 + 2048) * sizeof(int64_t)));
    return CFMM_OK;
}


int cfmm_clock_probe_start(cfmm_ctx *ctx, double period_us, double max_ms)
{
    if (!ctx || !(period_us >= 1.0) || !(max_ms > 0.0) || max_ms > 60000.0) return CFMM_E_ARG;
    HIP_TRY(ctx, hipSetDevice(ctx->device));
    { int rc_ = settle(ctx); if (rc_) return rc_; }
    if (ctx->probe_running) return fail(ctx, CFMM_E_STATE, "clock probe: already running (cfmm_clock_probe_stop first)");
    if (!ctx->probe_stream) HIP_TRY(ctx, hipStreamCreateWithFlags(&ctx->probe_stream, hipStreamNonBlocking));
    if (!ctx->probe_ring) {
        HIP_TRY(ctx, hipHostMalloc((void **)&ctx->probe_ring, (2 * PROBE_CAP + 8) * sizeof(long long), hipHostMallocMapped));
        HIP_TRY(ctx, hipHostGetDevicePointer((void **)&ctx->probe_ring_d, ctx->probe_ring, 0));
    }
    std::memset(ctx->probe_ring, 0, (2 * PROBE_CAP + 8) * sizeof(long long));
    hipLaunchKernelGGL(clock_probe_kernel, dim3(1), dim3(64), 0, ctx->probe_stream, ctx->probe_ring_d, PROBE_CAP,
                       (long long)(period_us * 100.0), (long long)(max_ms * 1e5));
    HIP_TRY(ctx, hipGetLastError());
    ctx->probe_running = true;
    return CFMM_OK;
}
int cfmm_clock_probe_read(cfmm_ctx *ctx, int64_t *out, int cap, int *count)
{
    if (!ctx || !count || (cap > 0 && !out)) return CFMM_E_ARG;
    *count = 0;
    if (!ctx->probe_ring) return CFMM_OK;
    const long long head = __atomic_load_n(reinterpret_cast<volatile long long *>(ctx->probe_ring) + 2 * PROBE_CAP + 1, __ATOMIC_ACQUIRE);
    const int k = (int)std::min<long long>(std::min<long long>(head, PROBE_CAP), cap);
    for (int i = 0; i < 2 * k; ++i) out[i] = reinterpret_cast<volatile long long *>(ctx->probe_ring)[i];
    *count = k;
    return CFMM_OK;
}
int cfmm_clock_probe_chain(cfmm_ctx *ctx, int64_t *out3)
{
    if (!ctx || !out3) return CFMM_E_ARG;
    for (int i = 0; i < 3; ++i) out3[i] = ctx->probe_ring ? reinterpret_cast<volatile long long *>(ctx->probe_ring)[2 * PROBE_CAP + 2 + i] : 0;
    return CFMM_OK;
}
int cfmm_clock_probe_stop(cfmm_ctx *ctx, int64_t *out, int cap, int *count)
{
    if (!ctx) return CFMM_E_ARG;
    if (ctx->probe_running) {
        HIP_TRY(ctx, hipSetDevice(ctx->device));
        __atomic_store_n(reinterpret_cast<volatile long long *>(ctx->probe_ring) + 2 * PROBE_CAP, 1ll, __ATOMIC_RELEASE);
        HIP_TRY(ctx, hipStreamSynchronize(ctx->probe_stream));
        ctx->probe_running = false;
    }
    int dummy = 0;
    return cfmm_clock_probe_read(ctx, out, cap, count ? count : &dummy);
}

int cfmm_time_xcd_handoff(cfmm_ctx *ctx, int np, int reps, double *out7)
{
    double *out6 = out7;
    if (!ctx || !out6 || np < 1 || np > 8192 || reps < 1) return CFMM_E_ARG;
    HIP_TRY(ctx, hipSetDevice(ctx->device));
    { int rc_ = settle(ctx); if (rc_) return rc_; }
    const int grid = ctx->cus;
    double *pub = nullptr; unsigned long long *flag = nullptr; long long *stamps = nullptr;
    HIP_TRY(ctx, hipMalloc(&pub, (size_t)16 * np * sizeof(double)));
    HIP_TRY(ctx, hipMalloc(&flag, 16 * 16 * sizeof(unsigned long long)));
    HIP_TRY(ctx, hipMalloc(&stamps, (size_t)4 * grid * sizeof(long long)));
    HIP_TRY(ctx, hipMemset(flag, 0, 16 * 16 * sizeof(unsigned long long)));
    (void)hipFuncSetAttribute((const void *)xcd_handoff_kernel, hipFuncAttributeMaxDynamicSharedMemorySize, 128 * 1024);
    std::vector<long long> h((size_t)4 * grid);
    std::vector<double> full, seen;
    int wrong_xcc = 0, failed = 0, orphan = 0;
    for (int r = 0; r < reps; ++r) {
        hipLaunchKernelGGL(xcd_handoff_kernel, dim3(grid), dim3(1024), (size_t)96 * 1024, ctx->stream, pub, flag, (unsigned long long)(r + 1), np, 500ll, stamps);
        HIP_TRY(ctx, hipGetLastError());
        HIP_TRY(ctx, hipMemcpyAsync(h.data(), stamps, h.size() * sizeof(long long), hipMemcpyDeviceToHost, ctx->stream));
        HIP_TRY(ctx, hipStreamSynchronize(ctx->stream));
        long long ready[16]; bool have[16] = {};
        for (int b = 0; b < 8 && b < grid; ++b) { const int x = (int)h[4 * b] & 15; ready[x] = h[4 * b + 1]; have[x] = true; }
        long long worst = 0, worst_seen = 0;
        wrong_xcc = 0; orphan = 0;
        for (int x = 0; x < 8; ++x) orphan += !have[x];
        for (int b = 0; b < grid; ++b) {
            const int x = (int)h[4 * b] & 15;
            wrong_xcc += x != b % 8;
            if (b < 8) continue;
            if (h[4 * b + 3] != 0 || !have[x]) { ++failed; continue; }
            worst = std::max(worst, h[4 * b + 2] - ready[x]);
            worst_seen = std::max(worst_seen, h[4 * b + 1] - ready[x]);
        }
        full.push_back(worst * 0.01); seen.push_back(worst_seen * 0.01);
    }
    std::sort(full.begin(), full.end()); std::sort(seen.begin(), seen.end());
    out6[0] = full[full.size() / 2]; out6[1] = full.back(); out6[2] = seen[seen.size() / 2];
    out6[3] = wrong_xcc; out6[4] = failed; out6[5] = orphan;
    out7[6] = 0.0;
    for (int b = 0; b < 8 && b < grid; ++b) out7[6] = 10.0 * out7[6] + (double)((int)h[4 * b] & 15 ? ((int)h[4 * b] & 15) % 10 : 0);
    (void)hipFree(pub); (void)hipFree(flag); (void)hipFree(stamps);
    return CFMM_OK;
}

int cfmm_time_eval_kernel(cfmm_ctx *ctx, int kind, int reps, double *sec_per_launch)
{
    if (!ctx || reps < 1 || !sec_per_launch) return CFMM_E_ARG;
    PoolEntry entry(ctx); HIP_TRY(ctx, entry.device);
    if (!ctx->pt.have_nu) return fail(ctx, CFMM_E_STATE, "time_eval_kernel: no prices set");
    HIP_TRY(ctx, hipMemcpyAsync(ctx->nu, ctx->nu_acc, ctx->n * sizeof(double), hipMemcpyDeviceToDevice, ctx->stream));
    HIP_TRY(ctx, hipMemsetAsync(ctx->nu + ctx->n, 0, sizeof(double), ctx->stream));
    const int only = kind == CFMM_TIME_ALL ? 0x7fffffff : kind;
    const bool table_only = kind == CFMM_TIME_TABLE;
    const EvalArgs ea = make_eval_args(ctx, false, only), es = make_eval_args(ctx, true, only);
    if (table_only ? table_pools(ctx) == 0 : ea.ntiles + es.ntiles == 0) return fail(ctx, CFMM_E_ARG, "time_eval_kernel: bucket %d is empty", kind);
    auto launch = [&]() {
        if (table_only) { launch_table_evals<false>(ctx, ctx->nu, ctx->acc); return; }
        launch_eval<false, false>(ctx, ea); launch_eval<false, true>(ctx, es);
        if (kind == CFMM_TIME_ALL && table_pools(ctx) > 0) launch_table_evals<false>(ctx, ctx->nu, ctx->acc);
    };
    for (int i = 0; i < 3; ++i) launch();
    HIP_TRY(ctx, hipEventRecord(ctx->ev_t0, ctx->stream));
    for (int i = 0; i < reps; ++i) launch();
    HIP_TRY(ctx, hipEventRecord(ctx->ev_t1, ctx->stream));
    HIP_TRY(ctx, hipMemsetAsync(ctx->acc, 0, (size_t)ctx->nslices * acc_stride(ctx->n) * sizeof(double), ctx->stream));
    if (ctx->det) HIP_TRY(ctx, hipMemsetAsync(ctx->acc_l, 0, 6 * (size_t)ctx->n * sizeof(unsigned long long), ctx->stream));
    HIP_TRY(ctx, hipStreamSynchronize(ctx->stream));
    HIP_TRY(ctx, hipGetLastError());
    float ms = 0.f;
    HIP_TRY(ctx, hipEventElapsedTime(&ms, ctx->ev_t0, ctx->ev_t1));
    *sec_per_launch = ms * 1e-3 / reps;
    return CFMM_OK;
}

int cfmm_time_newton_kernels(cfmm_ctx *ctx, double mu, int reps, double *out4)
{
    if (!ctx || reps < 1 || !out4 || !(mu > 0.0)) return CFMM_E_ARG;
    PoolEntry entry(ctx); HIP_TRY(ctx, entry.device);
    const char *why = "";
    if (!newton_supported(ctx, &why)) return fail(ctx, CFMM_E_UNSUPPORTED, "time_newton_kernels: %s", why);
    const int n = ctx->n, nr = hess_nr(n), ld = hess_ld(n);
    int rc = smooth_buffers(ctx, true); if (rc) return rc;
    if (!ctx->pt.have_nu) return fail(ctx, CFMM_E_STATE, "time_newton_kernels: no prices (cfmm_set_nu or a solve first)");
    HIP_TRY(ctx, hipMemcpyAsync(ctx->nu, ctx->nu_acc, n * sizeof(double), hipMemcpyDeviceToDevice, ctx->stream));
    HIP_TRY(ctx, hipMemsetAsync(ctx->sm_mask, 0, n * sizeof(int), ctx->stream));
    for (int k = 0; k < CFMM_POOL_KINDS2; ++k)
        if (ctx->sm_ws[k]) HIP_TRY(ctx, hipMemsetAsync(ctx->sm_ws[k], 0, 2 * (size_t)ctx->pools->r2[k].b.m * sizeof(double), ctx->stream));
    float ms = 0.f;
    for (int which = 0; which < 2; ++which) {
        if ((rc = launch_smooth(ctx, mu, which == 0, true, false))) return rc;
        HIP_TRY(ctx, hipEventRecord(ctx->ev_t0, ctx->stream));
        for (int i = 0; i < reps; ++i) if ((rc = launch_smooth(ctx, mu, which == 0, true, false))) return rc;
        HIP_TRY(ctx, hipEventRecord(ctx->ev_t1, ctx->stream));
        HIP_TRY(ctx, hipStreamSynchronize(ctx->stream));
        HIP_TRY(ctx, hipEventElapsedTime(&ms, ctx->ev_t0, ctx->ev_t1));
        out4[which] = ms * 1e-3 / reps;
    }
    if ((rc = launch_smooth(ctx, mu, true, true, false))) return rc;
    std::vector<double> hd(n, 0.0), rhs(n, 1.0);
    {
        std::vector<double> col(n);
        double mx = 0.0;
        for (int j = 0; j < n; j += std::max(1, n / 64)) {
            HIP_TRY(ctx, hipMemcpy(&col[j], ctx->H + (size_t)j * ld + j, sizeof(double), hipMemcpyDeviceToHost));
            mx = std::max(mx, std::fabs(col[j]));
        }
        for (int j = 0; j < n; ++j) hd[j] = 1e-3 * std::max(mx, 1e-300);
    }
    HIP_TRY(ctx, hipMemcpyAsync(ctx->sm_vec, hd.data(), n * sizeof(double), hipMemcpyHostToDevice, ctx->stream));
    HIP_TRY(ctx, hipMemcpyAsync(ctx->sm_vec + n, rhs.data(), n * sizeof(double), hipMemcpyHostToDevice, ctx->stream));
    hipLaunchKernelGGL(hess_finish_kernel, dim3(1024), dim3(256), 0, ctx->stream, ctx->H, n, nr, ld, (const double *)ctx->sm_vec,
                       (const int *)ctx->sm_mask, (const double *)(ctx->sm_vec + n));
    struct Scratch {
        double *keep = nullptr; hipEvent_t ev_end = nullptr;
        ~Scratch() { if (ev_end) (void)hipEventDestroy(ev_end); if (keep) (void)hipFree(keep); }
    } sc;
    HIP_TRY(ctx, hipMalloc((void **)&sc.keep, (size_t)ld * nr * sizeof(double)));
    double *const keep = sc.keep;
    HIP_TRY(ctx, hipMemcpyAsync(keep, ctx->H, (size_t)ld * nr * sizeof(double), hipMemcpyDeviceToDevice, ctx->stream));
    double fac = 0.0, back = 0.0;
    HIP_TRY(ctx, hipEventCreate(&sc.ev_end));
    const hipEvent_t ev_end = sc.ev_end;
    for (int i = 0; i < reps && rc == CFMM_OK; ++i) {
        if (hipMemcpyAsync(ctx->H, keep, (size_t)ld * nr * sizeof(double), hipMemcpyDeviceToDevice, ctx->stream) != hipSuccess) { rc = CFMM_E_HIP; break; }
        (void)hipEventRecord(ctx->ev_t0, ctx->stream);
        rc = launch_factor(ctx, n);
        (void)hipEventRecord(ctx->ev_t1, ctx->stream);
        if (rc == CFMM_OK) rc = launch_backsolve(ctx, n, ctx->sm_vec + n);
        (void)hipEventRecord(ev_end, ctx->stream);
        if (hipStreamSynchronize(ctx->stream) != hipSuccess) { rc = CFMM_E_HIP; break; }
        (void)hipEventElapsedTime(&ms, ctx->ev_t0, ctx->ev_t1); fac += ms * 1e-3;
        (void)hipEventElapsedTime(&ms, ctx->ev_t1, ev_end); back += ms * 1e-3;
    }
    drop_barrier(ctx);
    if (rc) { const std::string prev = ctx->err; return fail(ctx, rc, "time_newton_kernels: the factorisation launches failed (%s; %s)", prev.c_str(), hipGetErrorString(hipGetLastError())); }
    out4[2] = fac / reps; out4[3] = back / reps;
    return CFMM_OK;
}

int cfmm_time_collective(cfmm_ctx *ctx, int reps, double *fold_sec, double *allreduce_sec)
{
    if (!ctx || reps < 1) return CFMM_E_ARG;
    HIP_TRY(ctx, hipSetDevice(ctx->device));
    { int rc_ = settle(ctx); if (rc_) return rc_; }
    const int n = ctx->n, len = acc_arb(n) + 1;
    float ms = 0.f;
    HIP_TRY(ctx, hipMemsetAsync(ctx->acc, 0, (size_t)ctx->nslices * acc_stride(n) * sizeof(double), ctx->stream));
    const bool folded_inside = ctx->os_ready && (size_t)len <= ctx->os_cap && !ctx->det;
    cfmm_opts od; cfmm_default_opts(&od); od.memory = 3;
    const bool unfolded = rccl_unfolded(ctx) && fused_applies(ctx, od);
    if (fold_sec) *fold_sec = 0.0;
    if (!folded_inside && !unfolded) {
        HIP_TRY(ctx, hipEventRecord(ctx->ev_t0, ctx->stream));
        for (int i = 0; i < reps; ++i)
            hipLaunchKernelGGL(fold_kernel, dim3((len + 255) / 256), dim3(256), 0, ctx->stream, ctx->acc, n, ctx->nslices, 0, (const DevState *)nullptr);
        HIP_TRY(ctx, hipEventRecord(ctx->ev_t1, ctx->stream));
        HIP_TRY(ctx, hipStreamSynchronize(ctx->stream));
        HIP_TRY(ctx, hipEventElapsedTime(&ms, ctx->ev_t0, ctx->ev_t1));
        if (fold_sec) *fold_sec = ms * 1e-3 / reps;
    }
    if (allreduce_sec) *allreduce_sec = 0.0;
    if (sharded(ctx) && allreduce_sec) {
        const int fs = folded_inside ? ctx->nslices : 1;
        const size_t cnt = unfolded ? (size_t)(ctx->nslices - 1) * acc_stride(n) + len : (size_t)len;
        for (int i = 0; i < 3; ++i) { int rc = all_reduce(ctx, ctx->acc, cnt, NCCL_FLOAT64, NCCL_SUM, nullptr, fs); if (rc) return rc; }
        HIP_TRY(ctx, hipEventRecord(ctx->ev_t0, ctx->stream));
        for (int i = 0; i < reps; ++i) { int rc = all_reduce(ctx, ctx->acc, cnt, NCCL_FLOAT64, NCCL_SUM, nullptr, fs); if (rc) return rc; }
        HIP_TRY(ctx, hipEventRecord(ctx->ev_t1, ctx->stream));
        HIP_TRY(ctx, hipStreamSynchronize(ctx->stream));
        HIP_TRY(ctx, hipEventElapsedTime(&ms, ctx->ev_t0, ctx->ev_t1));
        *allreduce_sec = ms * 1e-3 / reps;
    }
    return CFMM_OK;
}

}
```

cfmm-routing-code_amd/csrc/iterate.hpp:

```cpp
#pragma once
#include <utility>
#include "kernels.hpp"

namespace cfmm {

#ifndef ITER_E_SMALL_DEF
#define ITER_E_SMALL_DEF 2
#endif
constexpr int ITER_E_SMALL = ITER_E_SMALL_DEF;
constexpr int ITER_MM = 3;
constexpr int ITER_P = ITER_MM + 1;
constexpr int GI_U = 8, GI_V = GI_U + ITER_P, GI_SY = GI_V + ITER_P, GI_YHY = GI_SY + ITER_P * (ITER_P - 1) / 2,
              GI_END = GI_YHY + ITER_P * (ITER_P + 1) / 2;
static_assert(GI_END <= 32, "the batch must fit one 32-value reduce-scatter");
constexpr int XS_HIST = 5;
constexpr int XS_VECS = XS_HIST + 2 * ITER_MM;
__host__ __device__ inline int iter_xvs(int n) { return (n + 3) & ~1; }

constexpr int ITER_HRING = 1024;
__host__ __device__ inline unsigned long long iter_hring_word(int evals, int status, int launch)
{
    return (unsigned long long)((unsigned)evals & 0xffffffu) | ((unsigned long long)((unsigned)status & 0xffu) << 24) | ((unsigned long long)(unsigned)launch << 32);
}
struct EnvRec {
    unsigned long long prog, seal;
    long long t0, t1;
};
struct IterArgs {
    EvalArgs ev;
    int n, M, nread, phase;
    int xvs, max_evals, pg_rule;
    int plain;
    double *acc3; long long acc_set;
    double *xs; long long xs_set;
    DevState *st3;
    const double *c, *h, *glo, *ghi;
    const int *ctype;
    double *Ds;
    double *nu, *nu_acc, *psi_acc;
    double tol_gap, tol_infeas, armijo, max_step;
    unsigned long long *hstat;
    unsigned long long *hring;
    int launch;
    double *h_nu_acc, *h_psi_acc;
    DevState *h_final;
    EnvRec *env;
    unsigned epoch;
};

template <int E> __device__ __forceinline__ void ldE(const double *p, int first, double (&v)[E]);
template <> __device__ __forceinline__ void ldE<1>(const double *p, int first, double (&v)[1]) { v[0] = p[first]; }
template <> __device__ __forceinline__ void ldE<2>(const double *p, int first, double (&v)[2])
{
    const double2 t = *reinterpret_cast<const double2 *>(p + first);
    v[0] = t.x; v[1] = t.y;
}
template <int E> __device__ __forceinline__ void ldEi(const int *p, int first, int (&v)[E]);
template <> __device__ __forceinline__ void ldEi<1>(const int *p, int first, int (&v)[1]) { v[0] = p[first]; }
template <> __device__ __forceinline__ void ldEi<2>(const int *p, int first, int (&v)[2])
{
    const int2 t = *reinterpret_cast<const int2 *>(p + first);
    v[0] = t.x; v[1] = t.y;
}
template <int E> __device__ __forceinline__ void stE(double *p, int first, int len, const double (&v)[E])
{
    if (E == 2 && first + 1 < len) { *reinterpret_cast<double2 *>(p + first) = make_double2(v[0], v[E - 1]); return; }
    if (first < len) p[first] = v[0];
}

template <int E> __device__ __forceinline__ void stX(double *p, int first, const double (&v)[E])
{
    if (E == 2) *reinterpret_cast<double2 *>(p + first) = make_double2(v[0], v[E - 1]);
    else p[first] = v[0];
}

template <int E>
struct GramIn {
    double g1[8];
    double S[ITER_P][E], Y[ITER_P][E], q0[E], H0[E], hq[E];
};
__host__ __device__ constexpr int sy_row(int c) { int k = 1; while (k * (k + 1) / 2 <= c) ++k; return k; }
__host__ __device__ constexpr int yhy_row(int c) { int k = 0; while ((k + 1) * (k + 2) / 2 <= c) ++k; return k; }
template <int I, int E>
__device__ __forceinline__ double gram_val(const GramIn<E> &in)
{
    double r = 0.0;
    if constexpr (I < GI_U) r = in.g1[I];
    else if constexpr (I < GI_V) {
#pragma unroll
        for (int e = 0; e < E; ++e) r = fma(in.S[I - GI_U][e], in.q0[e], r);
    } else if constexpr (I < GI_SY) {
#pragma unroll
        for (int e = 0; e < E; ++e) r = fma(in.Y[I - GI_V][e], in.hq[e], r);
    } else if constexpr (I < GI_YHY) {
        constexpr int c = I - GI_SY, k = sy_row(c), j = c - k * (k - 1) / 2;
        static_assert(j >= 0 && j < k && k < ITER_P, "SY index");
#pragma unroll
        for (int e = 0; e < E; ++e) r = fma(in.S[k][e], in.Y[j][e], r);
    } else if constexpr (I < GI_END) {
        constexpr int c = I - GI_YHY, k = yhy_row(c), j = c - k * (k + 1) / 2;
        static_assert(j >= 0 && j <= k && k < ITER_P, "YHY index");
#pragma unroll
        for (int e = 0; e < E; ++e) r = fma(in.H0[e] * in.Y[k][e], in.Y[j][e], r);
    }
    return r;
}

template <int I, int E>
__device__ __forceinline__ double gram_pair16(const GramIn<E> &in)
{
    const double a = gram_val<I, E>(in), b = gram_val<I + 16, E>(in);
    const int l0 = __double2loint(a), h0 = __double2hiint(a);
    const int l1 = __double2loint(b), h1 = __double2hiint(b);
    const auto lo = __builtin_amdgcn_permlane16_swap(l0, l1, false, false);
    const auto hi = __builtin_amdgcn_permlane16_swap(h0, h1, false, false);
    return __hiloint2double(hi[0], lo[0]) + __hiloint2double(hi[1], lo[1]);
}
template <int E, int... I>
__device__ __forceinline__ void gram_pairs16(const GramIn<E> &in, double (&v)[16], std::integer_sequence<int, I...>)
{
    ((v[I] = gram_pair16<I, E>(in)), ...);
}
__device__ __forceinline__ double row_halve4(double (&v)[8], int lane)
{
    const bool b4 = lane & 4, b2 = lane & 2, b1 = lane & 1;
#pragma unroll
    for (int i = 0; i < 4; ++i) {
        const double keep = b4 ? v[i + 4] : v[i], send = b4 ? v[i] : v[i + 4];
        v[i] = keep + swz_xor4(send);
    }
#pragma unroll
    for (int i = 0; i < 2; ++i) {
        const double keep = b2 ? v[i + 2] : v[i], send = b2 ? v[i] : v[i + 2];
        v[i] = keep + dpp_f64<0x4E>(send);
    }
    const double keep = b1 ? v[1] : v[0], send = b1 ? v[0] : v[1];
    return keep + dpp_f64<0xB1>(send);
}
template <int E>
__device__ __forceinline__ double gram_reduce32(const GramIn<E> &in, int lane)
{
    const bool b8 = lane & 8;
    double v[16];
    gram_pairs16<E>(in, v, std::make_integer_sequence<int, 16>{});
    double w[8];
#pragma unroll
    for (int i = 0; i < 8; ++i) {
        const double keep = b8 ? v[i + 8] : v[i], send = b8 ? v[i] : v[i + 8];
        w[i] = keep + dppd_ror8(send);
    }
    const double r = row_halve4(w, lane);
    double x, y;
    swap32_f64(r, x, y);
    return x + y;
}

template <int... I>
__device__ __forceinline__ int gram_selfcheck(const GramIn<1> &in, int lane, double q, std::integer_sequence<int, I...>)
{
    int bad = 0;
    (([&] {
        const double want = wave_allsum(gram_val<I, 1>(in));
        if ((lane & 31) == I && q != want) ++bad;
    }()), ...);
    return bad;
}
__global__ void __launch_bounds__(64)
selftest_gram_kernel(int *out)
{
    const int lane = threadIdx.x;
    GramIn<1> in;
#pragma unroll
    for (int i = 0; i < 8; ++i) in.g1[i] = (double)(((lane + 2) * (i + 3)) % 17) - 8.0;
#pragma unroll
    for (int k = 0; k < ITER_P; ++k) {
        in.S[k][0] = (double)(((lane + 5) * (k + 2)) % 11) - 5.0;
        in.Y[k][0] = (double)(((lane + 1) * (k + 7)) % 13) - 6.0;
    }
    in.q0[0] = (double)((lane * 7) % 9) - 4.0;
    in.H0[0] = (double)((lane % 3) + 1);
    in.hq[0] = in.H0[0] * in.q0[0];
    const double q = gram_reduce32<1>(in, lane);
    atomicAdd(out, gram_selfcheck(in, lane, q, std::make_integer_sequence<int, 32>{}));
}

__device__ __forceinline__ int uni(int v) { return __builtin_amdgcn_readfirstlane(v); }
__device__ __forceinline__ double uni(double v)
{
    return __hiloint2double(__builtin_amdgcn_readfirstlane(__double2hiint(v)), __builtin_amdgcn_readfirstlane(__double2loint(v)));
}

__host__ __device__ inline int iter_extra_lds_doubles(int n, bool dma = false)
{
    return (dma ? 2 * iter_xvs(n) + (STAGE_BYTES / 8) * (EVAL_THREADS / 64) : 4 * iter_xvs(n)) + 32;
}

template <int E, bool DET = false, bool PLAIN = false, bool DMA = false, int NT = 0>
__global__ void __launch_bounds__(EVAL_THREADS, EVAL_WAVES_PER_SIMD)
iter_kernel(IterArgs a)
{
    extern __shared__ __attribute__((aligned(16))) double lds_raw[];
    constexpr int SLOT = STAGE_BYTES / 8, NSLOT = EVAL_THREADS / 64;
    double *const stage0 = lds_raw;
    double *const lds = lds_raw + (DMA ? NSLOT * SLOT : 0);
    constexpr int MM = ITER_MM, P = ITER_P;
    static_assert(MM == 3, "DevState::rhow0..2 hold a window of 3");
    const int n = a.n, M = a.M;
    const int tid = threadIdx.x, lane = tid & 63, wave = uni((int)(threadIdx.x >> 6)), nw = blockDim.x >> 6;
    const int tile = eval_tile_doubles(n, DET);
    double *psi_s = lds;
    double *nu_s = lds + tile;
    double *fpart = nu_s + n + 2;
    int *next_tile = reinterpret_cast<int *>(fpart + 16);
    double *strips = lds + eval_lds_doubles(n, false, DET);
    constexpr bool LNU = eval_has_lnu(false, DET) && !DMA;
    double *lnu_s = lds + eval_lnu_offset(n, false, DET);
    double *xw = strips;
    double *xm = xw + 16 * 32;
    BlockRed red(xm + 32);
    double *ctl = xm + 32 + 2 * BlockRed::NRED * 16;
    int *ctli = reinterpret_cast<int *>(ctl + 2 * ITER_P + 2);
    double *gst_s = psi_s;
    double *sts_s = nu_s;
    double *glo_s = strips + 2 * 64 * (EVAL_THREADS / 64);
    double *ghi_s = glo_s + a.xvs;
    double *psi_k = DMA ? stage0 + NSLOT * SLOT - 2 * a.xvs : ghi_s + a.xvs, *nu_k = psi_k + a.xvs;
    double *fsafe = (DMA ? ghi_s : ghi_s + 2 * a.xvs) + a.xvs;
    const int first_late = (NSLOT * SLOT - 2 * a.xvs) / SLOT;

#ifdef CFMM_PHASE_TIMERS
    const long long ts_c16 = clock64(), ts_w16 = wall_clock64();
#endif
    const int p = a.phase, pr = (p + 2) % 3, pz = (p + 1) % 3;
    const int stride = acc_stride(n), xvs = a.xvs;
    const double *Xr = a.xs + (size_t)pr * a.xs_set;
    double *Xw = a.xs + (size_t)p * a.xs_set;
    const double *Ar = a.acc3 + (size_t)pr * a.acc_set;
    enum { R_STATE = 0, R_S = 0, R_ST = 1, R_GS = 2, R_D = 3, R_NU = 4, R_SW = 5, R_YW = 5 + ITER_MM, R_PSI_ACC = 5 + 2 * ITER_MM, R_NU_ACC, R_DS };
    const bool wide = gridDim.x > R_DS;
    const bool has_role = !wide || blockIdx.x <= R_DS;
    auto mine = [&](int role) { return wide ? blockIdx.x == (unsigned)role : blockIdx.x == (unsigned)role % gridDim.x; };
    const bool wr = mine(R_STATE);
    const int r0 = tid * E;
    const int ld0 = (r0 < n) ? r0 : 0;
    bool tin[E];
#pragma unroll
    for (int e = 0; e < E; ++e) tin[e] = r0 + e < n;
    const bool wave_active = wave * 64 * E < n;
    const int nwa = (n + 64 * E - 1) / (64 * E);
    red.nw = nwa;
    GramIn<E> in;
    double s[E], s_t[E], Gs[E], nuj[E], Ds[E], glo[E], ghi[E], hj[E], cj[E], psi[E];
    int ct[E];
#pragma unroll
    for (int e = 0; e < E; ++e) {
        s[e] = s_t[e] = Gs[e] = nuj[e] = Ds[e] = glo[e] = cj[e] = 0.0; psi[e] = 0.0; ghi[e] = __builtin_inf(); hj[e] = 0.0; ct[e] = 0;
        in.q0[e] = in.H0[e] = in.hq[e] = 0.0;
#pragma unroll
        for (int k = 0; k < P; ++k) { in.S[k][e] = 0.0; in.Y[k][e] = 0.0; }
    }
    if (wave_active) {
        ldE<E>(Xr, ld0, s); ldE<E>(Xr + xvs, ld0, s_t); ldE<E>(Xr + 2 * xvs, ld0, Gs); ldE<E>(Xr + 4 * xvs, ld0, nuj);
        ldE<E>(a.Ds, ld0, Ds); ldE<E>(a.glo, ld0, glo); ldE<E>(a.c, ld0, cj);
        if (!PLAIN) { ldE<E>(a.ghi, ld0, ghi); ldE<E>(a.h, ld0, hj); ldEi<E>(a.ctype, ld0, ct); }
        for (int sl = 0; sl < a.nread; ++sl) {
            double t1[E];
            ldE<E>(Ar + (size_t)sl * stride, ld0, t1);
#pragma unroll
            for (int e = 0; e < E; ++e) psi[e] += t1[e];
        }
#pragma unroll
        for (int k = 0; k < MM; ++k) {
            ldE<E>(Xr + (size_t)(XS_HIST + k) * xvs, ld0, in.S[k + 1]);
            ldE<E>(Xr + (size_t)(XS_HIST + MM + k) * xvs, ld0, in.Y[k + 1]);
        }
    }
    if (DET) for (int j = n + tid; j < tile; j += blockDim.x) psi_s[j] = 0.0;
    DevState st = a.st3[pr];
    if (st.status != 0) {
        if (blockIdx.x == 0 && tid == 0) {
            a.st3[p] = st;
            if (a.hring) __hip_atomic_store(a.hring + (a.launch & (ITER_HRING - 1)), iter_hring_word(st.evals, st.status, a.launch), __ATOMIC_RELAXED, __HIP_MEMORY_SCOPE_SYSTEM);
            if (a.env) {
                if (a.launch == st.evals + 1) a.env->t1 = wall_clock64();
                __hip_atomic_store(&a.env->seal, iter_hring_word(st.evals, st.status, (int)a.epoch), __ATOMIC_RELEASE, __HIP_MEMORY_SCOPE_SYSTEM);
            }
        }
        return;
    }
    st.evals = uni(st.evals); st.iters = uni(st.iters); st.first = uni(st.first); st.hist = uni(st.hist);
    st.nrej = uni(st.nrej); st.f = uni(st.f); st.t_step = uni(st.t_step);
    long long *const tsb = (st.evals + 1 < a.max_evals) ? a.ev.ts : nullptr;
    (void)tsb;
    PHASE_STAMP(tsb, 17);

    if (blockIdx.x == gridDim.x - 1) {
        double *Z = a.acc3 + (size_t)pz * a.acc_set;
        const int len = a.ev.nslices * stride;
        for (int j = tid; j < len; j += blockDim.x) Z[j] = 0.0;
    }

    bool act[E];
#pragma unroll
    for (int e = 0; e < E; ++e) act[e] = true;
    const bool keeps_acc = has_role && (mine(R_PSI_ACC) || mine(R_NU_ACC));
    if (wave_active) {
        double mx[2] = {0.0, 0.0};
        if (st.first) {
            double dg[E];
#pragma unroll
            for (int e = 0; e < E; ++e) dg[e] = 0.0;
            for (int sl = 0; sl < a.nread; ++sl) {
                double t2[E];
                ldE<E>(Ar + (size_t)sl * stride + acc_diag(n), ld0, t2);
#pragma unroll
                for (int e = 0; e < E; ++e) dg[e] += t2[e];
            }
#pragma unroll
            for (int e = 0; e < E; ++e) Ds[e] = dg[e];
            if (has_role && r0 < n && mine(R_DS)) stE<E>(a.Ds, r0, n, Ds);
        }
#pragma unroll
        for (int k = 0; k < MM; ++k) {
            const bool have = k < st.hist;
#pragma unroll
            for (int e = 0; e < E; ++e) if (!have || !tin[e]) { in.S[k + 1][e] = 0.0; in.Y[k + 1][e] = 0.0; }
        }
        double fpools = 0.0;
        if (tid < a.nread) fpools = Ar[(size_t)tid * stride + acc_arb(n)];
#pragma unroll
        for (int i = 0; i < 8; ++i) in.g1[i] = 0.0;
        in.g1[0] = fpools;
        double Gs_t[E];
#pragma unroll
        for (int e = 0; e < E; ++e) {
            Gs_t[e] = 0.0;
            if (tin[e]) {
                const double rj = PLAIN ? psi[e] : psi[e] + hj[e];
                Gs_t[e] = nuj[e] * rj;
                if (!PLAIN) in.g1[0] += (nuj[e] - cj[e]) * hj[e];
                in.g1[1] += (nuj[e] - cj[e]) * rj;
                mx[0] = fmax(mx[0], (PLAIN || ct[e] == 0) ? fmax(-rj, 0.0) : (ct[e] == 1 ? fabs(rj) : 0.0));
                mx[1] = fmax(mx[1], PLAIN ? fabs(psi[e]) : fmax(fabs(psi[e]), fabs(hj[e])));
                const double sv = s_t[e] - s[e], yv = Gs_t[e] - Gs[e];
                if (!st.first) {
                    in.S[0][e] = sv; in.Y[0][e] = yv;
                    in.g1[2] += Gs[e] * sv; in.g1[3] += Gs_t[e] * sv;
                    in.g1[4] += sv * yv; in.g1[5] += sv * sv; in.g1[6] += yv * yv;
                }
                const double G = Gs_t[e], sr = s_t[e];
                double v = G;
                if (!PLAIN && glo[e] == ghi[e]) v = 0.0;
                else if (sr <= glo[e] + 1e-14) v = fmin(G, 0.0);
                else if (!PLAIN && sr >= ghi[e] - 1e-14) v = fmax(G, 0.0);
                in.g1[7] += fabs(v);
                act[e] = PLAIN ? (sr <= glo[e] + 1e-14 && G > 0.0) : is_active(sr, glo[e], ghi[e], G);
                in.q0[e] = act[e] ? 0.0 : G;
                const double H = Ds[e] + fmax(G, 0.0);
                in.H0[e] = H > 0.0 ? rcp_nr(H) : 0.0;
                in.hq[e] = in.H0[e] * in.q0[e];
                gst_s[r0 + e] = Gs_t[e];
                sts_s[r0 + e] = s_t[e]; glo_s[r0 + e] = glo[e];
                if (!PLAIN) ghi_s[r0 + e] = ghi[e];
                if (keeps_acc) { psi_k[r0 + e] = psi[e]; nu_k[r0 + e] = nuj[e]; }
            }
        }
        PHASE_STAMP(tsb, 18);
        const double qa = gram_reduce32<E>(in, lane);
        PHASE_STAMP(tsb, 19);
        mx[0] = wave_allmax(mx[0]); mx[1] = wave_allmax(mx[1]);
        if (lane < 32) xw[wave * 32 + lane] = qa;
        if (lane == 0) { xm[wave * 2] = mx[0]; xm[wave * 2 + 1] = mx[1]; }
    }
    if (wave == nw - 1) build_tile_table(a.ev, next_tile, lane);
    __syncthreads();
    st.evals += 1;
    const bool keeps_acc0 = has_role && (mine(R_PSI_ACC) || mine(R_NU_ACC));
    const bool helper_mode = DMA && nwa < nw;
    if constexpr (DMA) {
        if (helper_mode && !wave_active && st.evals < a.max_evals) {
            __builtin_amdgcn_s_waitcnt(0x0F70);
            const int nhelp = nw - nwa, h = wave - nwa;
            for (int sl = h; sl < nw; sl += nhelp) {
                if (keeps_acc0 && sl >= first_late) continue;
                tiles_dma_first(a.ev, next_tile, lds_addr(stage0 + SLOT * sl), lane, sl);
            }
        }
    }

    bool accept = false, new_dir = false, pair_ok = false;
    double al[P], ga[P];
#pragma unroll
    for (int k = 0; k < P; ++k) { al[k] = 0.0; ga[k] = 0.0; }
    double gp_sq = 0.0;
    if (wave == 0) {
        double tl = 0.0;
        if (lane < 32) for (int w = 0; w < nwa; ++w) tl += xw[w * 32 + lane];
        const int tl_lo = __double2loint(tl), tl_hi = __double2hiint(tl);
        auto T = [&](int i) { return __hiloint2double(__builtin_amdgcn_readlane(tl_hi, i), __builtin_amdgcn_readlane(tl_lo, i)); };
        PHASE_STAMP(tsb, 20);
        double viol = 0.0, scale = 0.0;
        for (int w = 0; w < nwa; ++w) { viol = fmax(viol, xm[w * 2]); scale = fmax(scale, xm[w * 2 + 1]); }
        double rho[P];
        rho[0] = 0.0;
#pragma unroll
        for (int k = 0; k < MM; ++k) rho[k + 1] = (k < st.hist) ? uni(k == 0 ? st.rhow0 : (k == 1 ? st.rhow1 : st.rhow2)) : 0.0;
        const double f_t = T(0), gapv = T(1);

        accept = st.first != 0;
        if (!st.first) accept = lbfgs::accept(f_t, st.f, a.armijo, T(2), T(3));
        if (!accept) {
            lbfgs::reject(st);
        } else {
            const int old_hist0 = st.hist;
            if (!st.first) {
                const double sy = T(4);
                if (lbfgs::pair_ok(sy, T(5), T(6))) {
                    pair_ok = true;
                    rho[0] = rcp_nr(sy);
                    if (st.hist < M) st.hist += 1;
                }
                st.iters += 1;
            }
            gp_sq = T(7);
            lbfgs::certify(st, f_t, gapv, viol, scale, gp_sq);
            const bool was_first = st.first != 0;
            st.first = 0;
            if (lbfgs::converged(st, a.pg_rule, a.tol_gap, a.tol_infeas)) {
                st.status = 1;
            } else {
                new_dir = true;
                const int keep_old = lbfgs::keep_old(was_first, pair_ok, old_hist0, M);
#pragma unroll
                for (int k = 1; k < P; ++k) if (k - 1 >= keep_old) rho[k] = 0.0;
                lbfgs::gram_two_loop<P>(rho, [&](int k) { return T(GI_U + k); }, [&](int k) { return T(GI_V + k); },
                                        [&](int k, int j) { return T(GI_SY + k * (k - 1) / 2 + j); },
                                        [&](int k, int j) { return T(GI_YHY + k * (k + 1) / 2 + j); }, al, ga);
            }
            if (pair_ok) { st.rhow2 = st.rhow1; st.rhow1 = st.rhow0; st.rhow0 = rho[0]; }
        }
        if (lane == 0) {
#pragma unroll
            for (int k = 0; k < P; ++k) { ctl[k] = al[k]; ctl[P + k] = ga[k]; }
            ctl[2 * P] = st.t_step; ctl[2 * P + 1] = gp_sq;
            ctli[0] = accept ? 1 : 0; ctli[1] = new_dir ? 1 : 0; ctli[2] = st.status; ctli[3] = pair_ok ? 1 : 0;
        }
    }
    PHASE_STAMP(tsb, 21);
    if constexpr (DMA) lds_barrier(); else
    __syncthreads();
    accept = uni(ctli[0]) != 0; new_dir = uni(ctli[1]) != 0; pair_ok = uni(ctli[3]) != 0;
    gp_sq = uni(ctl[2 * P + 1]);
    if (wave != 0) { st.status = uni(ctli[2]); st.t_step = uni(ctl[2 * P]); }
    const bool dma_late = keeps_acc && wave >= first_late;
    if constexpr (DMA) {
        __builtin_amdgcn_s_waitcnt(0x0F70);
        if (!helper_mode && st.status == 0 && st.evals < a.max_evals && !dma_late) tiles_dma_first(a.ev, next_tile, lds_addr(stage0 + SLOT * wave), lane, wave);
    }
    if (new_dir && wave_active) {
#pragma unroll
        for (int k = 0; k < P; ++k) { al[k] = uni(ctl[k]); ga[k] = uni(ctl[P + k]); }
    }
    if (has_role && wave_active && r0 < n) {
        const int sh = (accept && pair_ok) ? 0 : 1;
#pragma unroll
        for (int k = 0; k < MM; ++k) {
            if (mine(R_SW + k)) { if (sh) stX<E>(Xw + (size_t)(XS_HIST + k) * xvs, r0, in.S[k + 1]); else stX<E>(Xw + (size_t)(XS_HIST + k) * xvs, r0, in.S[k]); }
            if (mine(R_YW + k)) { if (sh) stX<E>(Xw + (size_t)(XS_HIST + MM + k) * xvs, r0, in.Y[k + 1]); else stX<E>(Xw + (size_t)(XS_HIST + MM + k) * xvs, r0, in.Y[k]); }
        }
    }

    double d[E], v[E], nn[E];
#pragma unroll
    for (int e = 0; e < E; ++e) { s[e] = Gs[e] = d[e] = glo[e] = 0.0; ghi[e] = __builtin_inf(); v[e] = nn[e] = 0.0; }
    if (wave_active) {
#pragma unroll
        for (int e = 0; e < E; ++e) if (tin[e]) { glo[e] = glo_s[r0 + e]; if (!PLAIN) ghi[e] = ghi_s[r0 + e]; }
        if (accept) {
#pragma unroll
            for (int e = 0; e < E; ++e) if (tin[e]) { s[e] = sts_s[r0 + e]; Gs[e] = gst_s[r0 + e]; }
        } else {
            ldE<E>(Xr, ld0, s); ldE<E>(Xr + 2 * xvs, ld0, Gs); ldE<E>(Xr + 3 * xvs, ld0, d);
            if constexpr (DMA) __builtin_amdgcn_s_waitcnt(0x0F70);
        }
#pragma unroll
        for (int e = 0; e < E; ++e) if (tin[e]) psi_s[r0 + e] = 0.0;
        if (keeps_acc && accept && r0 < n) {
            double pk[E], nk[E];
#pragma unroll
            for (int e = 0; e < E; ++e) { pk[e] = tin[e] ? psi_k[r0 + e] : 0.0; nk[e] = tin[e] ? nu_k[r0 + e] : 0.0; }
            if (mine(R_PSI_ACC)) { stE<E>(a.psi_acc, r0, n, pk); if (a.h_psi_acc) stE<E>(a.h_psi_acc, r0, n, pk); }
            if (mine(R_NU_ACC)) { stE<E>(a.nu_acc, r0, n, nk); if (a.h_nu_acc) stE<E>(a.h_nu_acc, r0, n, nk); }
        }
    }

    auto trial = [&](double step) {
#pragma unroll
        for (int e = 0; e < E; ++e) {
            v[e] = fmax(s[e] + step * d[e], glo[e]);
            if (!PLAIN) v[e] = fmin(v[e], ghi[e]);
            nn[e] = tin[e] ? exp(v[e]) : 0.0;
        }
    };
    double F[2] = {0.0, 0.0};
    bool F_pending = false;
    auto safeguard = [&](double (&F)[2]) {
        bool redo = false;
        if (!(F[0] < 0.0) && gp_sq > 0.0) {
            st.hist = 0;
            double m1[1] = {0.0};
#pragma unroll
            for (int e = 0; e < E; ++e) {
                d[e] = (!tin[e] || act[e]) ? 0.0 : -Gs[e] * in.H0[e];
                m1[0] = fmax(m1[0], fabs(d[e]));
            }
            red.put<0, 1>(m1, wave_active);
            red.template get<0, 1, DMA>(m1);
            F[1] = m1[0];
            redo = true;
        }
        st.t_step = lbfgs::step_cap(F[1], a.max_step);
        const bool again = redo || st.t_step != 1.0;
        if (again && wave_active) trial(st.t_step);
        return again;
    };
    if (new_dir) {
        if (wave_active) {
#pragma unroll
            for (int e = 0; e < E; ++e) {
                double qm = in.q0[e], rs = 0.0;
#pragma unroll
                for (int k = 0; k < P; ++k) { qm -= al[k] * in.Y[k][e]; rs += ga[k] * in.S[k][e]; }
                d[e] = (tin[e] && !act[e]) ? -(in.H0[e] * qm + rs) : 0.0;
                F[0] += d[e] * Gs[e]; F[1] = fmax(F[1], fabs(d[e]));
            }
        }
#ifndef CFMM_EAGER_SAFEGUARD
        F_pending = st.evals < a.max_evals;
#endif
        if (F_pending) {
            if (wave_active) {
                F[0] = wave_allsum(F[0]); F[1] = wave_allmax(F[1]);
                if (lane == 0) { fsafe[wave] = F[0]; fsafe[16 + wave] = F[1]; }
                trial(1.0);
            }
        } else {
            red.put<1, 1>(F, wave_active);
            if (wave_active) trial(1.0);
            red.template get<1, 1, DMA>(F);
            (void)safeguard(F);
        }
    } else if (st.status == 0 && wave_active) trial(st.t_step);

    if (st.status == 0 && st.evals >= a.max_evals) st.status = 3;
    auto store_state = [&]() {
        if (has_role && wave_active && r0 < n) {
            if (mine(R_S)) stX<E>(Xw, r0, s);
            if (mine(R_ST)) stX<E>(Xw + xvs, r0, v);
            if (mine(R_GS)) stX<E>(Xw + 2 * xvs, r0, Gs);
            if (mine(R_D)) stX<E>(Xw + 3 * xvs, r0, d);
            if (mine(R_NU)) stX<E>(Xw + 4 * xvs, r0, nn);
            if (wr) stE<E>(a.nu, r0, n, nn);
        }
        if (wr) {
            if (tid == 0) {
                a.st3[p] = st; a.nu[n] = st.status != 0 ? 1.0 : 0.0;
                if (st.status != 0 && a.h_final) *a.h_final = st;
                if (a.env) __hip_atomic_store(&a.env->prog, iter_hring_word(st.evals, st.status, (int)a.epoch), __ATOMIC_RELAXED, __HIP_MEMORY_SCOPE_SYSTEM);
                else if (a.hstat) __hip_atomic_store(a.hstat, (unsigned long long)(unsigned)st.evals | ((unsigned long long)(unsigned)st.status << 32),
                                                __ATOMIC_RELAXED, __HIP_MEMORY_SCOPE_SYSTEM);
                if (a.hring) __hip_atomic_store(a.hring + (a.launch & (ITER_HRING - 1)), iter_hring_word(st.evals, st.status, a.launch), __ATOMIC_RELAXED, __HIP_MEMORY_SCOPE_SYSTEM);
            }
        }
    };
    if (st.status != 0) {
        store_state();
        if constexpr (DMA) dma_wait();
        return;
    }
    PHASE_STAMP(a.ev.ts, 22);
    auto publish = [&]() {
#pragma unroll
        for (int e = 0; e < E; ++e) if (tin[e]) { nu_s[r0 + e] = nn[e]; if constexpr (LNU) lnu_s[r0 + e] = v[e]; }
    };
    publish();
    if constexpr (DMA) {
        if (helper_mode && !wave_active) dma_wait();
        lds_barrier();
    } else
    __syncthreads();
    PHASE_STAMP(a.ev.ts, 23);
    if (F_pending) {
        F[0] = 0.0; F[1] = 0.0;
        for (int w = 0; w < nwa; ++w) { F[0] += fsafe[w]; F[1] = fmax(F[1], fsafe[16 + w]); }
        if (safeguard(F)) {
            publish();
            if constexpr (DMA) lds_barrier(); else __syncthreads();
        }
    }
    store_state();
#ifdef CFMM_PHASE_TIMERS
    if (a.ev.ts && tid == 0) {
        if (blockIdx.x == 0) { a.ev.ts[2 * 16] = ts_c16; a.ev.ts[2 * 16 + 1] = ts_w16; }
        if (blockIdx.x < 256) { long long *tb = a.ev.ts + 64 + 8 * 4096; tb[2 * blockIdx.x] = ts_w16; tb[2 * (blockIdx.x + 256)] = wall_clock64(); }
    }
#endif
    double2 *xs = reinterpret_cast<double2 *>(strips) + 64 * wave;
    if constexpr (DMA)
        eval_tiles_and_flush<false, false, DET, false, true, true>(a.ev, a.acc3 + (size_t)p * a.acc_set, nu_s, psi_s, nullptr, fpart, next_tile, xs,
                                                                   BatchCtl{1u, 0, 0}, nullptr, stage0 + SLOT * wave, !dma_late);
    else
    eval_tiles_and_flush<false, false, DET, false, true, false, NT, LNU>(a.ev, a.acc3 + (size_t)p * a.acc_set, nu_s, psi_s, nullptr, fpart, next_tile, xs,
                                                                         BatchCtl{1u, 0, 0}, nullptr, nullptr, false, lnu_s);
#ifdef CFMM_PHASE_TIMERS
    __syncthreads();
    if (a.ev.ts && tid == 0 && blockIdx.x < 256) a.ev.ts[64 + 8 * 4096 + 2 * blockIdx.x + 1] = wall_clock64();
#endif
}

}
```

Baseline: 48.52 billion pool-subproblems/s.

## Process four tokens per thread in iter kernel with LDS spill slots

Raises the default per-thread token count in the L-BFGS iteration kernel from 2 to 4 for small token counts. Each thread handles two pairs, and per-wave LDS slots stage the vectors of the second pair to limit register pressure. The Gram reduction gains a specialised four-element path that accumulates both halves before the tree reduction, and a new selftest covers it. This is meant to cut thread count and reduction work per token and improve ILP, at the cost of extra LDS traffic, larger LDS allocation and more complex indexing.

```diff
diff --git a/cfmm-routing-code_amd/csrc/cfmm_hip.hip b/cfmm-routing-code_amd/csrc/cfmm_hip.hip
--- a/cfmm-routing-code_amd/csrc/cfmm_hip.hip
+++ b/cfmm-routing-code_amd/csrc/cfmm_hip.hip
@@ -739,7 +739,7 @@
 {
     return (size_t)eval_lds_doubles(n, with_d, det) * sizeof(double) + (size_t)(EVAL_THREADS / 64) * 64 * 16 + (dma ? (size_t)(EVAL_THREADS / 64) * STAGE_BYTES : 0);
 }
-size_t iter_lds_bytes(int n, bool det = false, bool dma = false) { return eval_lds_bytes(n, false, det) + (size_t)iter_extra_lds_doubles(n, dma) * sizeof(double); }
+size_t iter_lds_bytes(int n, bool det = false, bool dma = false, bool e4 = false) { return eval_lds_bytes(n, false, det) + (size_t)iter_extra_lds_doubles(n, dma, e4) * sizeof(double); }
 constexpr size_t LDS_MAX = 160 * 1024;
 size_t upd_lds_bytes(int ng) { return (size_t)(2 * ng + 16 * 64 + 64 + 32 + 2 * 12 * 16 + 8) * sizeof(double); }
 
@@ -979,8 +979,11 @@
     if (ctx->n <= TINY_N && (rc = set_lds_attr(ctx, solve_tiny_kernel<false>, (size_t)tiny_lds_doubles(ctx->n) * sizeof(double)))) return rc;
     if (ctx->n <= TINY_N && (rc = set_lds_attr(ctx, solve_tiny_kernel<true>, (size_t)tiny_lds_doubles(ctx->n) * sizeof(double)))) return rc;
     const size_t il = iter_lds_bytes(ctx->n);
-    if ((rc = set_lds_attr(ctx, iter_kernel<ITER_E_SMALL, false, false>, il))) return rc;
-    if ((rc = set_lds_attr(ctx, iter_kernel<ITER_E_SMALL, false, true>, il))) return rc;
+    if (ITER_E_SMALL != 4 || iter_e4(ctx->n)) {
+        const size_t il4 = iter_lds_bytes(ctx->n, false, false, ITER_E_SMALL == 4);
+        if ((rc = set_lds_attr(ctx, iter_kernel<ITER_E_SMALL, false, false>, il4))) return rc;
+        if ((rc = set_lds_attr(ctx, iter_kernel<ITER_E_SMALL, false, true>, il4))) return rc;
+    }
     if ((rc = set_lds_attr(ctx, iter_kernel<2, false, false>, il))) return rc;
     if ((rc = set_lds_attr(ctx, iter_kernel<2, false, true>, il))) return rc;
     if ((rc = set_lds_attr(ctx, iter_kernel<2, false, false, false, 1>, il))) return rc;
@@ -1002,8 +1005,8 @@
         if ((rc = set_lds_attr(ctx, table_eval_kernel<false, true>, table_lds_bytes(ctx->n, false, true, GT_THREADS / 64)))) return rc;
         if ((rc = set_lds_attr(ctx, table_eval_kernel<true, true>, table_lds_bytes(ctx->n, true, true, GT_THREADS / 64)))) return rc;
         const size_t ild = iter_lds_bytes(ctx->n, true);
-        if ((rc = set_lds_attr(ctx, iter_kernel<ITER_E_SMALL, true, false>, ild))) return rc;
-        if ((rc = set_lds_attr(ctx, iter_kernel<ITER_E_SMALL, true, true>, ild))) return rc;
+        if ((rc = set_lds_attr(ctx, iter_kernel<ITER_E_DET, true, false>, ild))) return rc;
+        if ((rc = set_lds_attr(ctx, iter_kernel<ITER_E_DET, true, true>, ild))) return rc;
         if ((rc = set_lds_attr(ctx, iter_kernel<2, true, false>, ild))) return rc;
         if ((rc = set_lds_attr(ctx, iter_kernel<2, true, true>, ild))) return rc;
     }
@@ -1070,7 +1073,11 @@
     IterArgs a = base;
     a.phase = t % 3; a.launch = t;
     a.ev.rev = pingpong_on(ctx) ? (t & 1) : 0;
-    const int n = ctx->n, E = (n <= EVAL_THREADS && ITER_E_SMALL == 1) ? 1 : 2;
+    const bool dma = iter_dma(ctx);
+    const int big = dma ? 0 : large_set_mode(ctx);
+    const int n = ctx->n;
+    const int Es = (ITER_E_SMALL == 4) ? ((iter_e4(n) && !ctx->det && !dma && big == 0) ? 4 : 2) : (ctx->det ? ITER_E_DET : ITER_E_SMALL);
+    const int E = (n <= EVAL_THREADS) ? Es : 2;
     int grid, threads;
     {
         const int slots = ctx->cus * ctx->iter_blocks_per_cu * ctx->eval_grid_mult;
@@ -1083,9 +1090,7 @@
         if (grid > slots) grid = slots;
         if (grid < 1) grid = 1;
     }
-    const bool dma = iter_dma(ctx);
-    const int big = dma ? 0 : large_set_mode(ctx);
-    const size_t lds = iter_lds_bytes(n, ctx->det, dma);
+    const size_t lds = iter_lds_bytes(n, ctx->det, dma, E == 4);
     const dim3 g(grid), b(threads);
 #if CFMM_STAGED_WALK
 #define ITER_LAUNCH_DMA if (dma) { if (a.plain) hipLaunchKernelGGL((iter_kernel<2, false, true, true>), g, b, lds, ctx->stream, a); else hipLaunchKernelGGL((iter_kernel<2, false, false, true>), g, b, lds, ctx->stream, a); }
@@ -1095,9 +1100,9 @@
 #define ITER_LAUNCH(EE) do { \
         ITER_LAUNCH_DMA else if (big == 1) { if (a.plain) hipLaunchKernelGGL((iter_kernel<2, false, true, false, 1>), g, b, lds, ctx->stream, a); else hipLaunchKernelGGL((iter_kernel<2, false, false, false, 1>), g, b, lds, ctx->stream, a); } \
         else if (big == 2) { if (a.plain) hipLaunchKernelGGL((iter_kernel<2, false, true, false, 2>), g, b, lds, ctx->stream, a); else hipLaunchKernelGGL((iter_kernel<2, false, false, false, 2>), g, b, lds, ctx->stream, a); } \
-        else if (ctx->det) { if (a.plain) hipLaunchKernelGGL((iter_kernel<EE, true, true>), g, b, lds, ctx->stream, a); else hipLaunchKernelGGL((iter_kernel<EE, true, false>), g, b, lds, ctx->stream, a); } \
+        else if (ctx->det) { if (a.plain) hipLaunchKernelGGL((iter_kernel<(EE == 4 ? 2 : EE), true, true>), g, b, lds, ctx->stream, a); else hipLaunchKernelGGL((iter_kernel<(EE == 4 ? 2 : EE), true, false>), g, b, lds, ctx->stream, a); } \
         else { if (a.plain) hipLaunchKernelGGL((iter_kernel<EE, false, true>), g, b, lds, ctx->stream, a); else hipLaunchKernelGGL((iter_kernel<EE, false, false>), g, b, lds, ctx->stream, a); } } while (0)
-    if (E == 1) ITER_LAUNCH(ITER_E_SMALL); else ITER_LAUNCH(2);
+    if (E != 2) ITER_LAUNCH(ITER_E_SMALL); else ITER_LAUNCH(2);
 #undef ITER_LAUNCH
     double *acc_p = ctx->acc3 + (size_t)a.phase * acc_set_doubles(ctx);
     if (heavy_pools(ctx) > 0) {
@@ -4663,6 +4668,7 @@
     HIP_TRY(ctx, hipMemsetAsync(d, 0, sizeof(int), ctx->stream));
     hipLaunchKernelGGL(selftest_kernel, dim3(1), dim3(64), 0, ctx->stream, d);
     hipLaunchKernelGGL(selftest_gram_kernel, dim3(1), dim3(64), 0, ctx->stream, d);
+    hipLaunchKernelGGL(selftest_gram4_kernel, dim3(1), dim3(64), 0, ctx->stream, d);
     hipLaunchKernelGGL(selftest_log_kernel, dim3(1), dim3(64), 0, ctx->stream, d);
     hipLaunchKernelGGL(selftest_generic_kernel, dim3(1), dim3(64), 0, ctx->stream, d);
     hipLaunchKernelGGL(selftest_table_kernel, dim3(1), dim3(64), 0, ctx->stream, d);
diff --git a/cfmm-routing-code_amd/csrc/iterate.hpp b/cfmm-routing-code_amd/csrc/iterate.hpp
--- a/cfmm-routing-code_amd/csrc/iterate.hpp
+++ b/cfmm-routing-code_amd/csrc/iterate.hpp
@@ -5,9 +5,16 @@
 namespace cfmm {
 
 #ifndef ITER_E_SMALL_DEF
-#define ITER_E_SMALL_DEF 2
+#define ITER_E_SMALL_DEF 4
 #endif
 constexpr int ITER_E_SMALL = ITER_E_SMALL_DEF;
+static_assert(ITER_E_SMALL == 1 || ITER_E_SMALL == 2 || ITER_E_SMALL == 4, "ITER_E_SMALL_DEF");
+constexpr int ITER_E_DET = ITER_E_SMALL == 4 ? 2 : ITER_E_SMALL;
+constexpr int ITER_XVECS = 15;
+constexpr int ITER_XKEEP = 5;
+constexpr int ITER_XSLOT = (ITER_XVECS + ITER_XKEEP) * 128;
+constexpr int ITER_XWAVES = EVAL_THREADS / (64 * 4);
+__host__ __device__ inline bool iter_e4(int n) { return n <= 64 * 4 * ITER_XWAVES; }
 constexpr int ITER_MM = 3;
 constexpr int ITER_P = ITER_MM + 1;
 constexpr int GI_U = 8, GI_V = GI_U + ITER_P, GI_SY = GI_V + ITER_P, GI_YHY = GI_SY + ITER_P * (ITER_P - 1) / 2,
@@ -137,52 +144,103 @@
     const double keep = b1 ? v[1] : v[0], send = b1 ? v[0] : v[1];
     return keep + dpp_f64<0xB1>(send);
 }
-template <int E>
-__device__ __forceinline__ double gram_reduce32(const GramIn<E> &in, int lane)
+__device__ __forceinline__ void gram_halve8(const double (&v)[16], double (&w)[8], int lane)
 {
     const bool b8 = lane & 8;
-    double v[16];
-    gram_pairs16<E>(in, v, std::make_integer_sequence<int, 16>{});
-    double w[8];
 #pragma unroll
     for (int i = 0; i < 8; ++i) {
         const double keep = b8 ? v[i + 8] : v[i], send = b8 ? v[i] : v[i + 8];
         w[i] = keep + dppd_ror8(send);
     }
+}
+template <int I, bool ADD, int E>
+__device__ __forceinline__ void gram_pair8(const GramIn<E> &in, double (&w)[8], bool b8)
+{
+    const double lo = gram_pair16<I, E>(in), hi = gram_pair16<I + 8, E>(in);
+    const double keep = b8 ? hi : lo, send = b8 ? lo : hi;
+    const double t = keep + dppd_ror8(send);
+    w[I] = ADD ? w[I] + t : t;
+}
+template <bool ADD, int E, int... I>
+__device__ __forceinline__ void gram_pairs8(const GramIn<E> &in, double (&w)[8], int lane, std::integer_sequence<int, I...>)
+{
+    const bool b8 = lane & 8;
+    (gram_pair8<I, ADD, E>(in, w, b8), ...);
+}
+__device__ __forceinline__ double gram_tree8(double (&w)[8], int lane)
+{
     const double r = row_halve4(w, lane);
     double x, y;
     swap32_f64(r, x, y);
     return x + y;
 }
-
-template <int... I>
-__device__ __forceinline__ int gram_selfcheck(const GramIn<1> &in, int lane, double q, std::integer_sequence<int, I...>)
+__device__ __forceinline__ double gram_tree16(const double (&v)[16], int lane)
+{
+    double w[8];
+    gram_halve8(v, w, lane);
+    return gram_tree8(w, lane);
+}
+template <int E>
+__device__ __forceinline__ double gram_reduce32(const GramIn<E> &in, int lane)
+{
+    double v[16];
+    gram_pairs16<E>(in, v, std::make_integer_sequence<int, 16>{});
+    return gram_tree16(v, lane);
+}
+template <>
+__device__ __forceinline__ double gram_reduce32<4>(const GramIn<4> &in, int lane)
+{
+    double w[8];
+#pragma unroll
+    for (int q = 0; q < 2; ++q) {
+        GramIn<2> h;
+#pragma unroll
+        for (int i = 0; i < 8; ++i) h.g1[i] = q == 0 ? in.g1[i] : 0.0;
+#pragma unroll
+        for (int e = 0; e < 2; ++e) {
+            h.q0[e] = in.q0[2 * q + e]; h.H0[e] = in.H0[2 * q + e]; h.hq[e] = in.hq[2 * q + e];
+#pragma unroll
+            for (int k = 0; k < ITER_P; ++k) { h.S[k][e] = in.S[k][2 * q + e]; h.Y[k][e] = in.Y[k][2 * q + e]; }
+        }
+        if (q == 0) gram_pairs8<false, 2>(h, w, lane, std::make_integer_sequence<int, 8>{});
+        else gram_pairs8<true, 2>(h, w, lane, std::make_integer_sequence<int, 8>{});
+    }
+    return gram_tree8(w, lane);
+}
+
+template <int E, int... I>
+__device__ __forceinline__ int gram_selfcheck(const GramIn<E> &in, int lane, double q, std::integer_sequence<int, I...>)
 {
     int bad = 0;
     (([&] {
-        const double want = wave_allsum(gram_val<I, 1>(in));
+        const double want = wave_allsum(gram_val<I, E>(in));
         if ((lane & 31) == I && q != want) ++bad;
     }()), ...);
     return bad;
 }
-__global__ void __launch_bounds__(64)
-selftest_gram_kernel(int *out)
+template <int E>
+__device__ __forceinline__ void selftest_gram(int *out)
 {
     const int lane = threadIdx.x;
-    GramIn<1> in;
+    GramIn<E> in;
 #pragma unroll
     for (int i = 0; i < 8; ++i) in.g1[i] = (double)(((lane + 2) * (i + 3)) % 17) - 8.0;
 #pragma unroll
-    for (int k = 0; k < ITER_P; ++k) {
-        in.S[k][0] = (double)(((lane + 5) * (k + 2)) % 11) - 5.0;
-        in.Y[k][0] = (double)(((lane + 1) * (k + 7)) % 13) - 6.0;
-    }
-    in.q0[0] = (double)((lane * 7) % 9) - 4.0;
-    in.H0[0] = (double)((lane % 3) + 1);
-    in.hq[0] = in.H0[0] * in.q0[0];
-    const double q = gram_reduce32<1>(in, lane);
-    atomicAdd(out, gram_selfcheck(in, lane, q, std::make_integer_sequence<int, 32>{}));
-}
+    for (int e = 0; e < E; ++e) {
+#pragma unroll
+        for (int k = 0; k < ITER_P; ++k) {
+            in.S[k][e] = (double)(((lane + 5 + 3 * e) * (k + 2)) % 11) - 5.0;
+            in.Y[k][e] = (double)(((lane + 1 + 5 * e) * (k + 7)) % 13) - 6.0;
+        }
+        in.q0[e] = (double)(((lane + e) * 7) % 9) - 4.0;
+        in.H0[e] = (double)(((lane + e) % 3) + 1);
+        in.hq[e] = in.H0[e] * in.q0[e];
+    }
+    const double q = gram_reduce32<E>(in, lane);
+    atomicAdd(out, gram_selfcheck<E>(in, lane, q, std::make_integer_sequence<int, 32>{}));
+}
+__global__ void __launch_bounds__(64) selftest_gram_kernel(int *out) { selftest_gram<1>(out); }
+__global__ void __launch_bounds__(64) selftest_gram4_kernel(int *out) { selftest_gram<4>(out); }
 
 __device__ __forceinline__ int uni(int v) { return __builtin_amdgcn_readfirstlane(v); }
 __device__ __forceinline__ double uni(double v)
@@ -190,9 +248,10 @@
     return __hiloint2double(__builtin_amdgcn_readfirstlane(__double2hiint(v)), __builtin_amdgcn_readfirstlane(__double2loint(v)));
 }
 
-__host__ __device__ inline int iter_extra_lds_doubles(int n, bool dma = false)
-{
-    return (dma ? 2 * iter_xvs(n) + (STAGE_BYTES / 8) * (EVAL_THREADS / 64) : 4 * iter_xvs(n)) + 32;
+__host__ __device__ inline int iter_extra_lds_doubles(int n, bool dma = false, bool e4 = false)
+{
+    return (dma ? 2 * iter_xvs(n) + (STAGE_BYTES / 8) * (EVAL_THREADS / 64) : 4 * iter_xvs(n)) + 32
+           + (e4 ? ITER_XWAVES * ITER_XSLOT : 0);
 }
 
 template <int E, bool DET = false, bool PLAIN = false, bool DMA = false, int NT = 0>
@@ -202,7 +261,10 @@
     extern __shared__ __attribute__((aligned(16))) double lds_raw[];
     constexpr int SLOT = STAGE_BYTES / 8, NSLOT = EVAL_THREADS / 64;
     double *const stage0 = lds_raw;
-    double *const lds = lds_raw + (DMA ? NSLOT * SLOT : 0);
+    constexpr int EP = E == 4 ? 2 : E, NP = E / EP;
+    constexpr bool XD = NP == 2;
+    static_assert(!XD || (!DET && !DMA && NT == 0), "E = 4: default mode only");
+    double *const lds = lds_raw + (DMA ? NSLOT * SLOT : (XD ? ITER_XWAVES * ITER_XSLOT : 0));
     constexpr int MM = ITER_MM, P = ITER_P;
     static_assert(MM == 3, "DevState::rhow0..2 hold a window of 3");
     const int n = a.n, M = a.M;
@@ -243,36 +305,71 @@
     const bool wr = mine(R_STATE);
     const int r0 = tid * E;
     const int ld0 = (r0 < n) ? r0 : 0;
-    bool tin[E];
-#pragma unroll
-    for (int e = 0; e < E; ++e) tin[e] = r0 + e < n;
+    const int ld1 = (r0 + EP < n) ? r0 + EP : 0;
+    bool tin[NP][EP];
+#pragma unroll
+    for (int q = 0; q < NP; ++q)
+#pragma unroll
+        for (int e = 0; e < EP; ++e) tin[q][e] = r0 + q * EP + e < n;
     const bool wave_active = wave * 64 * E < n;
     const int nwa = (n + 64 * E - 1) / (64 * E);
     red.nw = nwa;
-    GramIn<E> in;
-    double s[E], s_t[E], Gs[E], nuj[E], Ds[E], glo[E], ghi[E], hj[E], cj[E], psi[E];
-    int ct[E];
-#pragma unroll
-    for (int e = 0; e < E; ++e) {
-        s[e] = s_t[e] = Gs[e] = nuj[e] = Ds[e] = glo[e] = cj[e] = 0.0; psi[e] = 0.0; ghi[e] = __builtin_inf(); hj[e] = 0.0; ct[e] = 0;
-        in.q0[e] = in.H0[e] = in.hq[e] = 0.0;
-#pragma unroll
-        for (int k = 0; k < P; ++k) { in.S[k][e] = 0.0; in.Y[k][e] = 0.0; }
-    }
+    GramIn<EP> in[NP];
+    double s[NP][EP], s_t[EP], Gs[NP][EP], nuj[EP], Ds[EP], glo[NP][EP], ghi[NP][EP], hj[EP], cj[EP], psi[NP][EP];
+    int ct[NP][EP];
+#pragma unroll
+    for (int q = 0; q < NP; ++q)
+#pragma unroll
+    for (int e = 0; e < EP; ++e) {
+        s[q][e] = Gs[q][e] = glo[q][e] = psi[q][e] = 0.0; ghi[q][e] = __builtin_inf(); ct[q][e] = 0;
+        s_t[e] = nuj[e] = Ds[e] = cj[e] = hj[e] = 0.0;
+        in[q].q0[e] = in[q].H0[e] = in[q].hq[e] = 0.0;
+#pragma unroll
+        for (int k = 0; k < P; ++k) { in[q].S[k][e] = 0.0; in[q].Y[k][e] = 0.0; }
+    }
+    const int xwave = XD && wave_active ? wave : 0;
+    double *const xslot = stage0 + ITER_XVECS * 128 * xwave + 2 * lane;
+    const int xkeep = uni(ITER_XVECS * 128 * ITER_XWAVES + (ITER_XKEEP - ITER_XVECS) * 128 * xwave);
+    auto xp = [&](int j) { return j < ITER_XVECS ? xslot + 128 * j : xslot + xkeep + 128 * (j - ITER_XVECS); };
+    auto xld = [&](int j, double (&v)[EP]) { const double2 t = *reinterpret_cast<const double2 *>(xp(j)); v[0] = t.x; v[EP - 1] = t.y; };
+    auto xst = [&](int j, const double (&v)[EP]) { *reinterpret_cast<double2 *>(xp(j)) = make_double2(v[0], v[EP - 1]); };
+    enum { X_S = 0, X_ST, X_GS, X_NU, X_DS, X_GLO, X_C, X_GHI, X_H, X_SW, X_YW = X_SW + ITER_MM, X_KEEP0 = X_YW + ITER_MM, X_END = X_KEEP0 + ITER_XKEEP,
+           XK_S0 = 0, XK_Y0, XK_Q0, XK_H0, XK_ACT };
+    static_assert(X_KEEP0 == ITER_XVECS && XK_ACT + 1 == ITER_XKEEP, "slot layout");
+    static_assert(!XD || ITER_XVECS * 1024 * ITER_XWAVES <= 65536, "LDS-DMA destinations travel through M0");
     if (wave_active) {
-        ldE<E>(Xr, ld0, s); ldE<E>(Xr + xvs, ld0, s_t); ldE<E>(Xr + 2 * xvs, ld0, Gs); ldE<E>(Xr + 4 * xvs, ld0, nuj);
-        ldE<E>(a.Ds, ld0, Ds); ldE<E>(a.glo, ld0, glo); ldE<E>(a.c, ld0, cj);
-        if (!PLAIN) { ldE<E>(a.ghi, ld0, ghi); ldE<E>(a.h, ld0, hj); ldEi<E>(a.ctype, ld0, ct); }
+        ldE<EP>(Xr, ld0, s[0]); ldE<EP>(Xr + xvs, ld0, s_t); ldE<EP>(Xr + 2 * xvs, ld0, Gs[0]); ldE<EP>(Xr + 4 * xvs, ld0, nuj);
+        ldE<EP>(a.Ds, ld0, Ds); ldE<EP>(a.glo, ld0, glo[0]); ldE<EP>(a.c, ld0, cj);
+        if (!PLAIN) { ldE<EP>(a.ghi, ld0, ghi[0]); ldE<EP>(a.h, ld0, hj); ldEi<EP>(a.ctype, ld0, ct[0]); }
         for (int sl = 0; sl < a.nread; ++sl) {
-            double t1[E];
-            ldE<E>(Ar + (size_t)sl * stride, ld0, t1);
-#pragma unroll
-            for (int e = 0; e < E; ++e) psi[e] += t1[e];
+            double t1[EP];
+            ldE<EP>(Ar + (size_t)sl * stride, ld0, t1);
+#pragma unroll
+            for (int e = 0; e < EP; ++e) psi[0][e] += t1[e];
         }
 #pragma unroll
         for (int k = 0; k < MM; ++k) {
-            ldE<E>(Xr + (size_t)(XS_HIST + k) * xvs, ld0, in.S[k + 1]);
-            ldE<E>(Xr + (size_t)(XS_HIST + MM + k) * xvs, ld0, in.Y[k + 1]);
+            ldE<EP>(Xr + (size_t)(XS_HIST + k) * xvs, ld0, in[0].S[k + 1]);
+            ldE<EP>(Xr + (size_t)(XS_HIST + MM + k) * xvs, ld0, in[0].Y[k + 1]);
+        }
+        if constexpr (XD) {
+            const unsigned sb = lds_addr(stage0 + ITER_XVECS * 128 * wave);
+            glds16(Xr + ld1, sb + 1024u * X_S); glds16(Xr + xvs + ld1, sb + 1024u * X_ST); glds16(Xr + 2 * xvs + ld1, sb + 1024u * X_GS);
+            glds16(Xr + 4 * xvs + ld1, sb + 1024u * X_NU);
+            glds16(a.Ds + ld1, sb + 1024u * X_DS); glds16(a.glo + ld1, sb + 1024u * X_GLO); glds16(a.c + ld1, sb + 1024u * X_C);
+            if (!PLAIN) { glds16(a.ghi + ld1, sb + 1024u * X_GHI); glds16(a.h + ld1, sb + 1024u * X_H); }
+#pragma unroll
+            for (int k = 0; k < MM; ++k) {
+                glds16(Xr + (size_t)(XS_HIST + k) * xvs + ld1, sb + 1024u * (X_SW + k));
+                glds16(Xr + (size_t)(XS_HIST + MM + k) * xvs + ld1, sb + 1024u * (X_YW + k));
+            }
+            if (!PLAIN) ldEi<EP>(a.ctype, ld1, ct[NP - 1]);
+            for (int sl = 0; sl < a.nread; ++sl) {
+                double t1[EP];
+                ldE<EP>(Ar + (size_t)sl * stride, ld1, t1);
+#pragma unroll
+                for (int e = 0; e < EP; ++e) psi[NP - 1][e] += t1[e];
+            }
         }
     }
     if (DET) for (int j = n + tid; j < tile; j += blockDim.x) psi_s[j] = 0.0;
@@ -286,10 +383,15 @@
                 __hip_atomic_store(&a.env->seal, iter_hring_word(st.evals, st.status, (int)a.epoch), __ATOMIC_RELEASE, __HIP_MEMORY_SCOPE_SYSTEM);
             }
         }
+        if constexpr (XD) dma_wait();
         return;
     }
     st.evals = uni(st.evals); st.iters = uni(st.iters); st.first = uni(st.first); st.hist = uni(st.hist);
     st.nrej = uni(st.nrej); st.f = uni(st.f); st.t_step = uni(st.t_step);
+    if constexpr (XD) {
+        st.head = uni(st.head); st.pad = uni(st.pad); st.gap = uni(st.gap); st.infeas = uni(st.infeas); st.primal = uni(st.primal); st.pg = uni(st.pg);
+        st.rhow0 = uni(st.rhow0); st.rhow1 = uni(st.rhow1); st.rhow2 = uni(st.rhow2);
+    }
     long long *const tsb = (st.evals + 1 < a.max_evals) ? a.ev.ts : nullptr;
     (void)tsb;
     PHASE_STAMP(tsb, 17);
@@ -300,73 +402,128 @@
         for (int j = tid; j < len; j += blockDim.x) Z[j] = 0.0;
     }
 
-    bool act[E];
-#pragma unroll
-    for (int e = 0; e < E; ++e) act[e] = true;
+    bool act[NP][EP];
+#pragma unroll
+    for (int q = 0; q < NP; ++q)
+#pragma unroll
+        for (int e = 0; e < EP; ++e) act[q][e] = true;
     const bool keeps_acc = has_role && (mine(R_PSI_ACC) || mine(R_NU_ACC));
+    const int hist0 = st.hist;
     if (wave_active) {
         double mx[2] = {0.0, 0.0};
-        if (st.first) {
-            double dg[E];
-#pragma unroll
-            for (int e = 0; e < E; ++e) dg[e] = 0.0;
-            for (int sl = 0; sl < a.nread; ++sl) {
-                double t2[E];
-                ldE<E>(Ar + (size_t)sl * stride + acc_diag(n), ld0, t2);
-#pragma unroll
-                for (int e = 0; e < E; ++e) dg[e] += t2[e];
-            }
-#pragma unroll
-            for (int e = 0; e < E; ++e) Ds[e] = dg[e];
-            if (has_role && r0 < n && mine(R_DS)) stE<E>(a.Ds, r0, n, Ds);
-        }
-#pragma unroll
-        for (int k = 0; k < MM; ++k) {
-            const bool have = k < st.hist;
-#pragma unroll
-            for (int e = 0; e < E; ++e) if (!have || !tin[e]) { in.S[k + 1][e] = 0.0; in.Y[k + 1][e] = 0.0; }
-        }
         double fpools = 0.0;
         if (tid < a.nread) fpools = Ar[(size_t)tid * stride + acc_arb(n)];
-#pragma unroll
-        for (int i = 0; i < 8; ++i) in.g1[i] = 0.0;
-        in.g1[0] = fpools;
-        double Gs_t[E];
-#pragma unroll
-        for (int e = 0; e < E; ++e) {
-            Gs_t[e] = 0.0;
-            if (tin[e]) {
-                const double rj = PLAIN ? psi[e] : psi[e] + hj[e];
-                Gs_t[e] = nuj[e] * rj;
-                if (!PLAIN) in.g1[0] += (nuj[e] - cj[e]) * hj[e];
-                in.g1[1] += (nuj[e] - cj[e]) * rj;
-                mx[0] = fmax(mx[0], (PLAIN || ct[e] == 0) ? fmax(-rj, 0.0) : (ct[e] == 1 ? fabs(rj) : 0.0));
-                mx[1] = fmax(mx[1], PLAIN ? fabs(psi[e]) : fmax(fabs(psi[e]), fabs(hj[e])));
-                const double sv = s_t[e] - s[e], yv = Gs_t[e] - Gs[e];
-                if (!st.first) {
-                    in.S[0][e] = sv; in.Y[0][e] = yv;
-                    in.g1[2] += Gs[e] * sv; in.g1[3] += Gs_t[e] * sv;
-                    in.g1[4] += sv * yv; in.g1[5] += sv * sv; in.g1[6] += yv * yv;
+        double run[8];
+#pragma unroll
+        for (int q = 0; q < NP; ++q) {
+            const int rq = r0 + q * EP, ldq = q == 0 ? ld0 : ld1;
+            GramIn<EP> &g = in[q];
+            if (q == 1) {
+                __builtin_amdgcn_sched_barrier(0);
+                dma_wait();
+            }
+            auto xin = [&](int e) {
+                asm volatile("" ::: "memory");
+                s[q][e] = xslot[128 * X_S + e]; s_t[e] = xslot[128 * X_ST + e]; Gs[q][e] = xslot[128 * X_GS + e]; nuj[e] = xslot[128 * X_NU + e];
+                glo[q][e] = xslot[128 * X_GLO + e]; cj[e] = xslot[128 * X_C + e];
+                if (!PLAIN) { ghi[q][e] = xslot[128 * X_GHI + e]; hj[e] = xslot[128 * X_H + e]; }
+            };
+            if (q == 1 && !st.first) xld(X_DS, Ds);
+            if (st.first) {
+                double dg[EP];
+#pragma unroll
+                for (int e = 0; e < EP; ++e) dg[e] = 0.0;
+                for (int sl = 0; sl < a.nread; ++sl) {
+                    double t2[EP];
+                    ldE<EP>(Ar + (size_t)sl * stride + acc_diag(n), ldq, t2);
+#pragma unroll
+                    for (int e = 0; e < EP; ++e) dg[e] += t2[e];
                 }
-                const double G = Gs_t[e], sr = s_t[e];
-                double v = G;
-                if (!PLAIN && glo[e] == ghi[e]) v = 0.0;
-                else if (sr <= glo[e] + 1e-14) v = fmin(G, 0.0);
-                else if (!PLAIN && sr >= ghi[e] - 1e-14) v = fmax(G, 0.0);
-                in.g1[7] += fabs(v);
-                act[e] = PLAIN ? (sr <= glo[e] + 1e-14 && G > 0.0) : is_active(sr, glo[e], ghi[e], G);
-                in.q0[e] = act[e] ? 0.0 : G;
-                const double H = Ds[e] + fmax(G, 0.0);
-                in.H0[e] = H > 0.0 ? rcp_nr(H) : 0.0;
-                in.hq[e] = in.H0[e] * in.q0[e];
-                gst_s[r0 + e] = Gs_t[e];
-                sts_s[r0 + e] = s_t[e]; glo_s[r0 + e] = glo[e];
-                if (!PLAIN) ghi_s[r0 + e] = ghi[e];
-                if (keeps_acc) { psi_k[r0 + e] = psi[e]; nu_k[r0 + e] = nuj[e]; }
-            }
-        }
-        PHASE_STAMP(tsb, 18);
-        const double qa = gram_reduce32<E>(in, lane);
+#pragma unroll
+                for (int e = 0; e < EP; ++e) Ds[e] = dg[e];
+                if (has_role && rq < n && mine(R_DS)) stE<EP>(a.Ds, rq, n, Ds);
+            }
+            if (q == 0) {
+#pragma unroll
+                for (int k = 0; k < MM; ++k) {
+                    const bool have = k < hist0;
+#pragma unroll
+                    for (int e = 0; e < EP; ++e) if (!have || !tin[q][e]) { g.S[k + 1][e] = 0.0; g.Y[k + 1][e] = 0.0; }
+                }
+            }
+#pragma unroll
+            for (int i = 0; i < 8; ++i) g.g1[i] = 0.0;
+            if (q == 0) g.g1[0] = fpools;
+            double Gs_t[EP];
+#pragma unroll
+            for (int e = 0; e < EP; ++e) {
+                Gs_t[e] = 0.0;
+                if (q == 1) xin(e);
+                if (tin[q][e]) {
+                    const double pe = psi[q][e];
+                    const double rj = PLAIN ? pe : pe + hj[e];
+                    Gs_t[e] = nuj[e] * rj;
+                    if (!PLAIN) g.g1[0] += (nuj[e] - cj[e]) * hj[e];
+                    g.g1[1] += (nuj[e] - cj[e]) * rj;
+                    mx[0] = fmax(mx[0], (PLAIN || ct[q][e] == 0) ? fmax(-rj, 0.0) : (ct[q][e] == 1 ? fabs(rj) : 0.0));
+                    mx[1] = fmax(mx[1], PLAIN ? fabs(pe) : fmax(fabs(pe), fabs(hj[e])));
+                    const double sv = s_t[e] - s[q][e], yv = Gs_t[e] - Gs[q][e];
+                    if (!st.first) {
+                        g.S[0][e] = sv; g.Y[0][e] = yv;
+                        g.g1[2] += Gs[q][e] * sv; g.g1[3] += Gs_t[e] * sv;
+                        g.g1[4] += sv * yv; g.g1[5] += sv * sv; g.g1[6] += yv * yv;
+                    }
+                    const double G = Gs_t[e], sr = s_t[e];
+                    double v = G;
+                    if (!PLAIN && glo[q][e] == ghi[q][e]) v = 0.0;
+                    else if (sr <= glo[q][e] + 1e-14) v = fmin(G, 0.0);
+                    else if (!PLAIN && sr >= ghi[q][e] - 1e-14) v = fmax(G, 0.0);
+                    g.g1[7] += fabs(v);
+                    act[q][e] = PLAIN ? (sr <= glo[q][e] + 1e-14 && G > 0.0) : is_active(sr, glo[q][e], ghi[q][e], G);
+                    g.q0[e] = act[q][e] ? 0.0 : G;
+                    const double H = Ds[e] + fmax(G, 0.0);
+                    g.H0[e] = H > 0.0 ? rcp_nr(H) : 0.0;
+                    g.hq[e] = g.H0[e] * g.q0[e];
+                    gst_s[rq + e] = Gs_t[e];
+                    sts_s[rq + e] = s_t[e]; glo_s[rq + e] = glo[q][e];
+                    if (!PLAIN) ghi_s[rq + e] = ghi[q][e];
+                    if (keeps_acc) { psi_k[rq + e] = pe; nu_k[rq + e] = nuj[e]; }
+                }
+            }
+            if (q == 1) {
+                asm volatile("" ::: "memory");
+#pragma unroll
+                for (int k = 0; k < MM; ++k) {
+                    xld(X_SW + k, g.S[k + 1]); xld(X_YW + k, g.Y[k + 1]);
+                    const bool have = k < hist0;
+#pragma unroll
+                    for (int e = 0; e < EP; ++e) if (!have || !tin[q][e]) { g.S[k + 1][e] = 0.0; g.Y[k + 1][e] = 0.0; }
+                }
+            }
+            if (q == 0) PHASE_STAMP(tsb, 18);
+            if constexpr (XD) {
+                if (q == 0) gram_pairs8<false, EP>(g, run, lane, std::make_integer_sequence<int, 8>{});
+                else gram_pairs8<true, EP>(g, run, lane, std::make_integer_sequence<int, 8>{});
+            } else {
+                double pv[16];
+                gram_pairs16<EP>(g, pv, std::make_integer_sequence<int, 16>{});
+                gram_halve8(pv, run, lane);
+            }
+            if constexpr (XD) {
+                const int kb = q == 0 ? X_KEEP0 : 0;
+                double af[EP];
+#pragma unroll
+                for (int e = 0; e < EP; ++e) af[e] = act[q][e] ? 1.0 : 0.0;
+                xst(kb + XK_S0, g.S[0]); xst(kb + XK_Y0, g.Y[0]); xst(kb + XK_Q0, g.q0); xst(kb + XK_H0, g.H0); xst(kb + XK_ACT, af);
+#pragma unroll
+                for (int e = 0; e < EP; ++e) {
+                    g.q0[e] = g.H0[e] = 0.0;
+#pragma unroll
+                    for (int k = 0; k < P; ++k) { g.S[k][e] = 0.0; g.Y[k][e] = 0.0; }
+                }
+            }
+        }
+        const double qa = gram_tree8(run, lane);
         PHASE_STAMP(tsb, 19);
         mx[0] = wave_allmax(mx[0]); mx[1] = wave_allmax(mx[1]);
         if (lane < 32) xw[wave * 32 + lane] = qa;
@@ -375,6 +532,15 @@
     if (wave == nw - 1) build_tile_table(a.ev, next_tile, lane);
     __syncthreads();
     st.evals += 1;
+    if constexpr (XD) {
+        if (wave_active) {
+#pragma unroll
+            for (int k = 0; k < MM; ++k) {
+                ldE<EP>(Xr + (size_t)(XS_HIST + k) * xvs, ld0, in[0].S[k + 1]);
+                ldE<EP>(Xr + (size_t)(XS_HIST + MM + k) * xvs, ld0, in[0].Y[k + 1]);
+            }
+        }
+    }
     const bool keeps_acc0 = has_role && (mine(R_PSI_ACC) || mine(R_NU_ACC));
     const bool helper_mode = DMA && nwa < nw;
     if constexpr (DMA) {
@@ -461,48 +627,81 @@
 #pragma unroll
         for (int k = 0; k < P; ++k) { al[k] = uni(ctl[k]); ga[k] = uni(ctl[P + k]); }
     }
-    if (has_role && wave_active && r0 < n) {
-        const int sh = (accept && pair_ok) ? 0 : 1;
-#pragma unroll
-        for (int k = 0; k < MM; ++k) {
-            if (mine(R_SW + k)) { if (sh) stX<E>(Xw + (size_t)(XS_HIST + k) * xvs, r0, in.S[k + 1]); else stX<E>(Xw + (size_t)(XS_HIST + k) * xvs, r0, in.S[k]); }
-            if (mine(R_YW + k)) { if (sh) stX<E>(Xw + (size_t)(XS_HIST + MM + k) * xvs, r0, in.Y[k + 1]); else stX<E>(Xw + (size_t)(XS_HIST + MM + k) * xvs, r0, in.Y[k]); }
-        }
-    }
-
-    double d[E], v[E], nn[E];
-#pragma unroll
-    for (int e = 0; e < E; ++e) { s[e] = Gs[e] = d[e] = glo[e] = 0.0; ghi[e] = __builtin_inf(); v[e] = nn[e] = 0.0; }
+    double d[NP][EP], v[NP][EP], nn[NP][EP];
+#pragma unroll
+    for (int q = 0; q < NP; ++q)
+#pragma unroll
+        for (int e = 0; e < EP; ++e) { s[q][e] = Gs[q][e] = d[q][e] = glo[q][e] = 0.0; ghi[q][e] = __builtin_inf(); v[q][e] = nn[q][e] = 0.0; }
+    double F[2] = {0.0, 0.0};
     if (wave_active) {
 #pragma unroll
-        for (int e = 0; e < E; ++e) if (tin[e]) { glo[e] = glo_s[r0 + e]; if (!PLAIN) ghi[e] = ghi_s[r0 + e]; }
-        if (accept) {
-#pragma unroll
-            for (int e = 0; e < E; ++e) if (tin[e]) { s[e] = sts_s[r0 + e]; Gs[e] = gst_s[r0 + e]; }
-        } else {
-            ldE<E>(Xr, ld0, s); ldE<E>(Xr + 2 * xvs, ld0, Gs); ldE<E>(Xr + 3 * xvs, ld0, d);
-            if constexpr (DMA) __builtin_amdgcn_s_waitcnt(0x0F70);
-        }
-#pragma unroll
-        for (int e = 0; e < E; ++e) if (tin[e]) psi_s[r0 + e] = 0.0;
-        if (keeps_acc && accept && r0 < n) {
-            double pk[E], nk[E];
-#pragma unroll
-            for (int e = 0; e < E; ++e) { pk[e] = tin[e] ? psi_k[r0 + e] : 0.0; nk[e] = tin[e] ? nu_k[r0 + e] : 0.0; }
-            if (mine(R_PSI_ACC)) { stE<E>(a.psi_acc, r0, n, pk); if (a.h_psi_acc) stE<E>(a.h_psi_acc, r0, n, pk); }
-            if (mine(R_NU_ACC)) { stE<E>(a.nu_acc, r0, n, nk); if (a.h_nu_acc) stE<E>(a.h_nu_acc, r0, n, nk); }
+        for (int q = 0; q < NP; ++q) {
+            const int rq = r0 + q * EP, ldq = q == 0 ? ld0 : ld1;
+            GramIn<EP> &g = in[q];
+            if constexpr (XD) {
+                const int kb = q == 0 ? X_KEEP0 : 0;
+                double af[EP];
+                xld(kb + XK_S0, g.S[0]); xld(kb + XK_Y0, g.Y[0]); xld(kb + XK_Q0, g.q0); xld(kb + XK_H0, g.H0); xld(kb + XK_ACT, af);
+#pragma unroll
+                for (int e = 0; e < EP; ++e) act[q][e] = af[e] != 0.0;
+#pragma unroll
+                for (int k = 0; k < MM; ++k) {
+                    if (q == 1) { xld(X_SW + k, g.S[k + 1]); xld(X_YW + k, g.Y[k + 1]); }
+                    const bool have = k < hist0;
+#pragma unroll
+                    for (int e = 0; e < EP; ++e) if (!have || !tin[q][e]) { g.S[k + 1][e] = 0.0; g.Y[k + 1][e] = 0.0; }
+                }
+            }
+            if (has_role && rq < n) {
+                const int sh = (accept && pair_ok) ? 0 : 1;
+#pragma unroll
+                for (int k = 0; k < MM; ++k) {
+                    if (mine(R_SW + k)) { if (sh) stX<EP>(Xw + (size_t)(XS_HIST + k) * xvs, rq, g.S[k + 1]); else stX<EP>(Xw + (size_t)(XS_HIST + k) * xvs, rq, g.S[k]); }
+                    if (mine(R_YW + k)) { if (sh) stX<EP>(Xw + (size_t)(XS_HIST + MM + k) * xvs, rq, g.Y[k + 1]); else stX<EP>(Xw + (size_t)(XS_HIST + MM + k) * xvs, rq, g.Y[k]); }
+                }
+            }
+#pragma unroll
+            for (int e = 0; e < EP; ++e) if (!XD && tin[q][e]) { glo[q][e] = glo_s[rq + e]; if (!PLAIN) ghi[q][e] = ghi_s[rq + e]; }
+            if (accept) {
+#pragma unroll
+                for (int e = 0; e < EP; ++e) if (tin[q][e]) { s[q][e] = sts_s[rq + e]; Gs[q][e] = gst_s[rq + e]; }
+            } else {
+                ldE<EP>(Xr, ldq, s[q]); ldE<EP>(Xr + 2 * xvs, ldq, Gs[q]); ldE<EP>(Xr + 3 * xvs, ldq, d[q]);
+                if constexpr (DMA) __builtin_amdgcn_s_waitcnt(0x0F70);
+            }
+#pragma unroll
+            for (int e = 0; e < EP; ++e) if (tin[q][e]) psi_s[rq + e] = 0.0;
+            if (keeps_acc && accept && rq < n) {
+                double pk[EP], nk[EP];
+#pragma unroll
+                for (int e = 0; e < EP; ++e) { pk[e] = tin[q][e] ? psi_k[rq + e] : 0.0; nk[e] = tin[q][e] ? nu_k[rq + e] : 0.0; }
+                if (mine(R_PSI_ACC)) { stE<EP>(a.psi_acc, rq, n, pk); if (a.h_psi_acc) stE<EP>(a.h_psi_acc, rq, n, pk); }
+                if (mine(R_NU_ACC)) { stE<EP>(a.nu_acc, rq, n, nk); if (a.h_nu_acc) stE<EP>(a.h_nu_acc, rq, n, nk); }
+            }
+            if (new_dir) {
+#pragma unroll
+                for (int e = 0; e < EP; ++e) {
+                    double qm = g.q0[e], rs = 0.0;
+#pragma unroll
+                    for (int k = 0; k < P; ++k) { qm -= al[k] * g.Y[k][e]; rs += ga[k] * g.S[k][e]; }
+                    d[q][e] = (tin[q][e] && !act[q][e]) ? -(g.H0[e] * qm + rs) : 0.0;
+                    F[0] += d[q][e] * Gs[q][e]; F[1] = fmax(F[1], fabs(d[q][e]));
+                }
+            }
         }
     }
 
     auto trial = [&](double step) {
 #pragma unroll
-        for (int e = 0; e < E; ++e) {
-            v[e] = fmax(s[e] + step * d[e], glo[e]);
-            if (!PLAIN) v[e] = fmin(v[e], ghi[e]);
-            nn[e] = tin[e] ? exp(v[e]) : 0.0;
+        for (int q = 0; q < NP; ++q)
+#pragma unroll
+        for (int e = 0; e < EP; ++e) {
+            if (XD && tin[q][e]) { glo[q][e] = glo_s[r0 + q * EP + e]; if (!PLAIN) ghi[q][e] = ghi_s[r0 + q * EP + e]; }
+            v[q][e] = fmax(s[q][e] + step * d[q][e], glo[q][e]);
+            if (!PLAIN) v[q][e] = fmin(v[q][e], ghi[q][e]);
+            nn[q][e] = tin[q][e] ? exp(v[q][e]) : 0.0;
         }
     };
-    double F[2] = {0.0, 0.0};
     bool F_pending = false;
     auto safeguard = [&](double (&F)[2]) {
         bool redo = false;
@@ -510,9 +709,11 @@
             st.hist = 0;
             double m1[1] = {0.0};
 #pragma unroll
-            for (int e = 0; e < E; ++e) {
-                d[e] = (!tin[e] || act[e]) ? 0.0 : -Gs[e] * in.H0[e];
-                m1[0] = fmax(m1[0], fabs(d[e]));
+            for (int q = 0; q < NP; ++q)
+#pragma unroll
+            for (int e = 0; e < EP; ++e) {
+                d[q][e] = (!tin[q][e] || act[q][e]) ? 0.0 : -Gs[q][e] * in[q].H0[e];
+                m1[0] = fmax(m1[0], fabs(d[q][e]));
             }
             red.put<0, 1>(m1, wave_active);
             red.template get<0, 1, DMA>(m1);
@@ -525,16 +726,6 @@
         return again;
     };
     if (new_dir) {
-        if (wave_active) {
-#pragma unroll
-            for (int e = 0; e < E; ++e) {
-                double qm = in.q0[e], rs = 0.0;
-#pragma unroll
-                for (int k = 0; k < P; ++k) { qm -= al[k] * in.Y[k][e]; rs += ga[k] * in.S[k][e]; }
-                d[e] = (tin[e] && !act[e]) ? -(in.H0[e] * qm + rs) : 0.0;
-                F[0] += d[e] * Gs[e]; F[1] = fmax(F[1], fabs(d[e]));
-            }
-        }
 #ifndef CFMM_EAGER_SAFEGUARD
         F_pending = st.evals < a.max_evals;
 #endif
@@ -554,13 +745,18 @@
 
     if (st.status == 0 && st.evals >= a.max_evals) st.status = 3;
     auto store_state = [&]() {
-        if (has_role && wave_active && r0 < n) {
-            if (mine(R_S)) stX<E>(Xw, r0, s);
-            if (mine(R_ST)) stX<E>(Xw + xvs, r0, v);
-            if (mine(R_GS)) stX<E>(Xw + 2 * xvs, r0, Gs);
-            if (mine(R_D)) stX<E>(Xw + 3 * xvs, r0, d);
-            if (mine(R_NU)) stX<E>(Xw + 4 * xvs, r0, nn);
-            if (wr) stE<E>(a.nu, r0, n, nn);
+        if (has_role && wave_active) {
+#pragma unroll
+            for (int q = 0; q < NP; ++q) {
+                const int rq = r0 + q * EP;
+                if (rq >= n) continue;
+                if (mine(R_S)) stX<EP>(Xw, rq, s[q]);
+                if (mine(R_ST)) stX<EP>(Xw + xvs, rq, v[q]);
+                if (mine(R_GS)) stX<EP>(Xw + 2 * xvs, rq, Gs[q]);
+                if (mine(R_D)) stX<EP>(Xw + 3 * xvs, rq, d[q]);
+                if (mine(R_NU)) stX<EP>(Xw + 4 * xvs, rq, nn[q]);
+                if (wr) stE<EP>(a.nu, rq, n, nn[q]);
+            }
         }
         if (wr) {
             if (tid == 0) {
@@ -581,7 +777,9 @@
     PHASE_STAMP(a.ev.ts, 22);
     auto publish = [&]() {
 #pragma unroll
-        for (int e = 0; e < E; ++e) if (tin[e]) { nu_s[r0 + e] = nn[e]; if constexpr (LNU) lnu_s[r0 + e] = v[e]; }
+        for (int q = 0; q < NP; ++q)
+#pragma unroll
+            for (int e = 0; e < EP; ++e) if (tin[q][e]) { nu_s[r0 + q * EP + e] = nn[q][e]; if constexpr (LNU) lnu_s[r0 + q * EP + e] = v[q][e]; }
     };
     publish();
     if constexpr (DMA) {
```

Result: slower. 40.69 billion pool-subproblems/s (-16.1%).
